# lijx10/SO-Net

Measured on AMD Instinct MI355X. Metric: point-clouds/sec forward, ModelNet40 5k-pt 8x8 SOM, higher is better.
Workload: dtype f32 (operands split into fp16 pieces, 3 fp16 MFMAs per product, f32 accumulate; parity 1e-5)

## Files before the change

### include/sonet_hip.h

```cpp
#ifndef SONET_HIP_H
#define SONET_HIP_H

#include <stddef.h>
#include <stdint.h>

#ifdef __cplusplus
extern "C" {
#endif

typedef void *sonet_stream_t;

enum {
    SONET_OK = 0,
    SONET_ERR_INVALID_ARG = 1,
    SONET_ERR_UNSUPPORTED = 2,
    SONET_ERR_LAUNCH = 3,
    SONET_ERR_NO_DEVICE = 4
};

int sonet_abi_version(void);
const char *sonet_build_arch(void);
const char *sonet_last_error(void);
int sonet_check_device(void);
int sonet_diag_mfma_f16_rate(int random_operands, int iters, double *tflops_out, double *ghz_out, sonet_stream_t stream);

int sonet_range_log_set(uint32_t *slot);

int sonet_index_max_f32(const float *data, const int32_t *index, int32_t *out_idx,
                        int B, int C, int Np, int K, sonet_stream_t stream);
int sonet_index_max_bf16(const uint16_t *data, const int32_t *index, int32_t *out_idx,
                         int B, int C, int Np, int K, sonet_stream_t stream);
int sonet_index_max_gather_f32(const float *data, const int32_t *index, const int32_t *row_max,
                               int32_t *out_idx, float *out_val,
                               int B, int C, int Np, int K, sonet_stream_t stream);
int sonet_index_max_gather_bf16(const uint16_t *data, const int32_t *index, const int32_t *row_max,
                                int32_t *out_idx, float *out_val, int B, int C, int Np, int K,
                                sonet_stream_t stream);
int sonet_index_max_gather_p16(const void *planes, const int32_t *index, const int32_t *row_max,
                               int32_t *out_idx, float *out_val, int B, int C, int Np, int K, sonet_stream_t stream);

int sonet_som_assign_f32(const float *x, const float *node, int B, int N, int M, int k,
                         int32_t *min_idx_i32, int64_t *min_idx_i64, int32_t *count, double *sum_ws,
                         sonet_stream_t stream);

int sonet_som_group_f32(const float *x, const float *sn, const int32_t *min_idx_i32,
                        const int32_t *count, const double *sum_ws, int B, int N, int M, int k,
                        float *som_node, int32_t *row_max, float *centers, float *x_decentered,
                        float *x_augmented, sonet_stream_t stream);

#define SONET_SOM_TRAIN_MAX_NODES 1024
#define SONET_SOM_TRAIN_MAX_POINTS (1 << 28)
int sonet_som_train_f32(const float *x, const float *node0, int node0_shared, const float *w, const float *lr,
                        int T, int B, int N, int M, float *node_out, sonet_stream_t stream);

int sonet_som_mask_i32(const int32_t *min_idx_i32, int32_t *mask, int B, int kN, int M,
                       sonet_stream_t stream);

int sonet_node_gather_f32(const float *feat, const int32_t *min_idx_i32, float *out,
                          int B, int C, int M, int kN, sonet_stream_t stream);

int sonet_knn_gather_f32(const float *x, const int64_t *knn_I, float *out,
                         int B, int C, int M, int K, sonet_stream_t stream);

int sonet_knn_self_f32(const float *node, int64_t *knn_I, int B, int M, int K, sonet_stream_t stream);

#define SONET_BATCH_SHAPENET 1
#define SONET_BATCH_TRAIN 2
#define SONET_BATCH_ROT_HORIZONTAL 4
#define SONET_BATCH_ROT_PERTURBATION 8
#define SONET_BATCH_TRANSLATION 16
#define SONET_BATCH_FLAG_MASK 31
#define SONET_BATCH_DRAW_SCALARS 8
#define SONET_BATCH_MAX_K 16
int sonet_assemble_batch_f32(const float *src, long long P, const int64_t *offsets, int S, const float *nodes_src,
                             const int64_t *idx, int B, int N, int M, int K, int flags, long long seed,
                             long long step, const int64_t *replay_idx, const double *replay_draws, double *draws_out,
                             float *pc, float *sn, float *node, int64_t *chosen, int64_t *knn_I, int32_t *bad,
                             sonet_stream_t stream);

int sonet_knn_group_f32(const float *coord, const float *feat, const int64_t *knn_I, int B, int C, int M, int K,
                        int center_avg, float *center, float *out, sonet_stream_t stream);
int sonet_knn_prepare_f32(const float *coord, const int64_t *knn_I, int B, int M, int K, int center_avg,
                          float *center, float *dec, int32_t *gidx, sonet_stream_t stream);
int sonet_pointmlp_h3_gather_f32(const float *x1, int C1, int L1, const int32_t *gidx, const float *x2, int C2, const void *Wp3,
                                 const float *scale, const float *shift, int relu, float *y,
                                 int B, int Cout, int L, sonet_stream_t stream);
int sonet_planes_max_f32(const float *x, float *out, long long rows, int K, int M, sonet_stream_t stream);

int sonet_lastdim_max_f32(const float *x, float *out, long long rows, int K, sonet_stream_t stream);

size_t sonet_pointmlp_pack_size(int Cin, int Cout);
int sonet_pointmlp_pack_f32(const float *W, float *Wp, int Cin, int Cout, sonet_stream_t stream);
int sonet_pointmlp_f32(const float *x1, int C1, const float *x2, int C2, const float *Wp,
                       const float *scale, const float *shift, int relu, float *y,
                       int B, int Cout, int L, sonet_stream_t stream);

int sonet_pointmlp_x3_bnb_f32(const float *gy, const float *raw, int C, const void *Wp3, const float *scale, const float *shift,
                              const float *a, const float *b, const float *c0, const float *sc, const float *sh, int relu,
                              float *g_raw_out, float *y, int B, int Cout, int L,
                              const float *praw, const float *psc, const float *psh, int prelu, void *pstats_ws, double *psums,
                              sonet_stream_t stream);

int sonet_pointmlp_x3_bnb_acc_f32(const float *gy, const float *raw, int C, const void *Wp3, const float *scale, const float *shift,
                                  const float *a, const float *b, const float *c0, const float *sc, const float *sh, int relu,
                                  float *g_raw_out, const float *yadd, float *y, int B, int Cout, int L, sonet_stream_t stream);

size_t sonet_pointmlp_x3_pack_size(int Cin, int Cout);
int sonet_pointmlp_x3_pack(const float *W, void *Wp3, int Cin, int Cout, sonet_stream_t stream);
int sonet_pointmlp_x3_f32(const float *x1, int C1, const float *x2, int C2, const void *Wp3,
                          const float *scale, const float *shift, int relu, float *y,
                          int B, int Cout, int L, sonet_stream_t stream);

int sonet_pointmlp_h3_pack(const float *W, void *Wp3, int Cin, int Cout, sonet_stream_t stream);
int sonet_pointmlp_h3_f32(const float *x1, int C1, const float *x2, int C2, const void *Wp3,
                          const float *scale, const float *shift, int relu, float *y,
                          int B, int Cout, int L, sonet_stream_t stream);

size_t sonet_p16_size(int B, int C, int L);
int sonet_p16_from_f32(const float *x, void *p16, int B, int C, int L, const float *scale, const float *shift, int relu,
                       sonet_stream_t stream);
int sonet_p16_to_f32(const void *p16, float *x, int B, int C, int L, sonet_stream_t stream);
size_t sonet_pointmlp_h3p_pack_size(int Cin, int Cout);
int sonet_pointmlp_h3p_pack(const float *W, void *Wp, int Cin, int Cout, sonet_stream_t stream);
size_t sonet_pointmlp_h3p_stats_ws_size(int B, int Cout, int L);
int sonet_pointmlp_h3p(const void *x1p, int C1, int L1, const int32_t *gidx, const void *x2p, int C2, const void *Wp,
                       const float *scale, const float *shift, int relu, float *y, void *yp, int B, int Cout, int L,
                       const float *zadd, const int32_t *zidx, int ZM, void *stats_ws, float *mean, float *var,
                       sonet_stream_t stream);

size_t sonet_knn_stage_columns(int B, int M, int K);
size_t sonet_node_stage_columns(int B, int M);
int sonet_knn_stage_prepare_f32(const float *coord, const int64_t *knn_I, int KI, int center_avg, int B, int M, int K,
                                float *center, void *center_p16, void *rec, sonet_stream_t stream);
int sonet_knn_stage_input_p16(const void *rec, const void *z_p16, const float *wl, const float *scale, const float *shift, int relu,
                              int B, int M, int K, int C, void *h1_p16, sonet_stream_t stream);
int sonet_pointmlp_h3p_gmax(const void *x1p, int C1, const void *x2p, int C2, const void *Wp, const float *scale, const float *shift,
                            int relu, int Cout, int L, int GK, int G, int ngout, int Lout, float *y, void *yp, sonet_stream_t stream);
int sonet_p16_flat_to_bcm_f32(const void *p16, float *x, int B, int C, int M, sonet_stream_t stream);

int sonet_lastdim_argmax_f32(const float *x, float *out, int32_t *idx, long long rows, int K, sonet_stream_t stream);
int sonet_lastdim_argmax_bf16(const uint16_t *x, uint16_t *out, int32_t *idx, long long rows, int K, sonet_stream_t stream);
int sonet_lastdim_max_bwd_f32(const float *g, const int32_t *idx, float *gx, long long rows, int K, sonet_stream_t stream);
int sonet_lastdim_max_bwd_bf16(const uint16_t *g, const int32_t *idx, uint16_t *gx, long long rows, int K, sonet_stream_t stream);
size_t sonet_knn_gather_bwd_ws_size(int B, int M, int K);
int sonet_knn_gather_bwd_f32(const float *g, const int64_t *knn_I, float *gx, void *ws, int B, int C, int M, int K, sonet_stream_t stream);
int sonet_knn_gather_bwd_bf16(const uint16_t *g, const int64_t *knn_I, float *gx, void *ws, int B, int C, int M, int K, sonet_stream_t stream);
size_t sonet_node_gather_bwd_ws_size(int B, int M, int L);
int sonet_node_gather_bwd_f32(const float *g, const int32_t *ids, float *gx, void *ws, int B, int C, int M, int L, sonet_stream_t stream);
int sonet_node_gather_bwd_bf16(const uint16_t *g, const int32_t *ids, float *gx, void *ws, int B, int C, int M, int L, sonet_stream_t stream);

size_t sonet_pointmlp_bf16_pack_size(int Cin, int Cout);
int sonet_pointmlp_bf16_pack(const float *W, void *Wp, int Cin, int Cout, sonet_stream_t stream);
int sonet_pointmlp_bf16(const uint16_t *x1, int C1, const uint16_t *x2, int C2, const void *Wp,
                        const float *scale, const float *shift, int relu, uint16_t *y,
                        int B, int Cout, int L, sonet_stream_t stream);
int sonet_pointmlp_bf16_gather(const uint16_t *x1, int C1, int L1, const int32_t *gidx, const uint16_t *x2, int C2, const void *Wp,
                               const float *scale, const float *shift, int relu, uint16_t *y,
                               int B, int Cout, int L, sonet_stream_t stream);
int sonet_pointmlp_bf16_acc(const uint16_t *x1, int C1, const uint16_t *x2, int C2, const void *Wp,
                            const float *scale, const float *shift, int relu, const uint16_t *yadd, uint16_t *y,
                            int B, int Cout, int L, sonet_stream_t stream);
int sonet_pointmlp_bf16_bnb(const uint16_t *gy, const uint16_t *raw, int C, const void *Wp, const float *scale, const float *shift,
                            const float *a, const float *b, const float *c0, const float *sc, const float *sh, int relu,
                            uint16_t *g_raw_out, const uint16_t *yadd, uint16_t *y, int B, int Cout, int L, sonet_stream_t stream);

size_t sonet_pointresnet_pack_size(void);
int sonet_pointresnet_pack(const float *W1, const float *W2, const float *W3, const float *W4, int Cin0,
                           void *wstream, sonet_stream_t stream);
int sonet_pointresnet_fused_f32(const float *x, int Cin0, const void *wstream, const float *affine,
                                float *y, int B, int L, sonet_stream_t stream);
int sonet_pointresnet_fused_p16_f32(const float *x, int Cin0, const void *wstream, const float *affine,
                                    float *y, void *yp, int B, int L, sonet_stream_t stream);

size_t sonet_pointresnet_bf16_pack_size(void);
int sonet_pointresnet_bf16_pack(const float *W1, const float *W2, const float *W3, const float *W4, int Cin0,
                                void *wstream, sonet_stream_t stream);
int sonet_pointresnet_bf16(const float *x, int Cin0, const void *wstream, const float *affine,
                           uint16_t *y, int B, int L, sonet_stream_t stream);

size_t sonet_pointresnet_bf16_pool_ws_size(int B, int L, int M);
int sonet_pointresnet_bf16_pool(const float *x_sorted, int Cin0, const void *wstream, const float *affine,
                                const int32_t *ids_sorted, const int32_t *pos0, const int32_t *node_off,
                                const int32_t *count, void *ws, float *out, int B, int L, int M, sonet_stream_t stream);

size_t sonet_pointresnet_pool_ws_size(int B, int L, int M);
int sonet_pointresnet_fused_pool_f32(const float *x_sorted, int Cin0, const void *wstream, const float *affine,
                                     const int32_t *ids_sorted, const int32_t *pos0, const int32_t *node_off,
                                     const int32_t *count, void *ws, float *out, int B, int L, int M, sonet_stream_t stream);
int sonet_pointresnet_fused_pool_p16_f32(const float *x_sorted, int Cin0, const void *wstream, const float *affine,
                                         const int32_t *ids_sorted, const int32_t *pos0, const int32_t *node_off,
                                         const int32_t *count, void *ws, float *out, void *out_p16, int B, int L, int M, sonet_stream_t stream);
size_t sonet_som_assign_sort_ws_size(int B, int N, int M, int k);
int sonet_som_assign_sort_f32(const float *x, const float *sn, const float *node, int B, int N, int M, int k,
                              int32_t *min_idx_i32, int64_t *min_idx_i64, int32_t *count, double *sum_ws,
                              float *som_node, int32_t *row_max, float *x_aug_sorted, int32_t *ids_sorted,
                              int32_t *pos0, int32_t *node_off, void *ws, sonet_stream_t stream);
int sonet_som_assign_sort_det_f32(const float *x, const float *sn, const float *node, int B, int N, int M, int k,
                              int32_t *min_idx_i32, int64_t *min_idx_i64, int32_t *count, double *sum_ws,
                              float *som_node, int32_t *row_max, float *x_aug_sorted, int32_t *ids_sorted,
                              int32_t *pos0, int32_t *node_off, void *ws, sonet_stream_t stream);
int sonet_som_assign_sort_knn_f32(const float *x, const float *sn, const float *node, int B, int N, int M, int k,
                                  int32_t *min_idx_i32, int64_t *min_idx_i64, int32_t *count, double *sum_ws,
                                  float *som_node, int32_t *row_max, float *x_aug_sorted, int32_t *ids_sorted,
                                  int32_t *pos0, int32_t *node_off, void *ws,
                                  const int64_t *knn_I, int KI, int K, int center_avg, float *center, void *center_p16, void *rec,
                                  sonet_stream_t stream);
int sonet_som_sort_group_f32(const float *x, const float *sn, const int32_t *min_idx_i32, const int32_t *count,
                             const double *sum_ws, int B, int N, int M, int k, float *som_node, int32_t *row_max,
                             float *x_aug_sorted, int32_t *ids_sorted, int32_t *pos0, int32_t *node_off,
                             int32_t *cursor_ws, sonet_stream_t stream);

int sonet_channel_stats_bf16(const uint16_t *y, int B, int C, int L, double *stat_ws, float *mean, float *var, sonet_stream_t stream);
int sonet_channel_affine_act_out_bf16(const uint16_t *x, const float *scale, const float *shift, int relu, uint16_t *y,
                                      int B, int C, int L, sonet_stream_t stream);
int sonet_pointwise_bwd_stats_bf16(const uint16_t *gy, const uint16_t *raw, const float *scale, const float *shift,
                                   int relu, int B, int C, int L, double *sums, sonet_stream_t stream);
int sonet_pointwise_bwd_apply_bf16(const uint16_t *gy, const uint16_t *raw, const float *scale, const float *shift, int relu,
                                   const float *a, const float *b, const float *c0, uint16_t *g_raw, int B, int C, int L,
                                   sonet_stream_t stream);

int sonet_pointwise_bwd_stats_f32(const float *gy, const float *raw, const float *scale, const float *shift,
                                  int relu, int B, int C, int L, double *sums, sonet_stream_t stream);
int sonet_pointwise_bwd_apply_f32(const float *gy, const float *raw, const float *scale, const float *shift, int relu,
                                  const float *a, const float *b, const float *c0, float *g_raw,
                                  int B, int C, int L, sonet_stream_t stream);
int sonet_node_add_affine_act_f32(float *t, const float *z, const int32_t *min_idx_i32, const float *scale,
                                  const float *shift, int relu, int B, int C, int L, int M, sonet_stream_t stream);

size_t sonet_pointmlp_stats_ws_size(int B, int Cout, int L);
int sonet_pointmlp_h3_stats_f32(const float *x1, int C1, const float *x2, int C2, const void *Wp3, const float *scale,
                                const float *shift, int relu, float *y, int B, int Cout, int L, void *stats_ws,
                                float *mean, float *var, sonet_stream_t stream);
int sonet_pointmlp_x3_stats_f32(const float *x1, int C1, const float *x2, int C2, const void *Wp3, const float *scale,
                                const float *shift, int relu, float *y, int B, int Cout, int L, void *stats_ws,
                                float *mean, float *var, sonet_stream_t stream);

int sonet_pointmlp_h3_nodeadd_f32(const float *x1, int C1, const float *x2, int C2, const void *Wp3, const float *scale,
                                  const float *shift, int relu, float *y, int B, int Cout, int L,
                                  const float *zadd, const int32_t *zidx, int ZM, sonet_stream_t stream);

size_t sonet_pointmlp_bf16_stats_ws_size(int B, int Cout, int L);
int sonet_pointmlp_bf16_stats(const uint16_t *x1, int C1, const uint16_t *x2, int C2, const void *Wp,
                              const float *scale, const float *shift, int relu, uint16_t *y,
                              int B, int Cout, int L, void *stats_ws, float *mean, float *var, sonet_stream_t stream);
int sonet_pointmlp_bf16_pool(const uint16_t *x1, int C1, const uint16_t *x2, int C2, const void *Wp,
                             const float *scale, const float *shift, int relu, const int32_t *ids, const int32_t *row_max,
                             int32_t *out_idx, float *out_val, int B, int Cout, int L, int M, sonet_stream_t stream);
int sonet_pointmlp_bf16_stats_xaff(const uint16_t *x1, int C1, const uint16_t *x2, int C2, const void *Wp,
                                   const float *scale, const float *shift, int relu, uint16_t *y,
                                   int B, int Cout, int L, void *stats_ws, float *mean, float *var,
                                   const float *xs1, const float *xh1, const float *xs2, const float *xh2, int xrelu,
                                   sonet_stream_t stream);
int sonet_pointmlp_bf16_pool_xaff(const uint16_t *x1, int C1, const uint16_t *x2, int C2, const void *Wp,
                                  const float *scale, const float *shift, int relu, const int32_t *ids, const int32_t *row_max,
                                  int32_t *out_idx, float *out_val, int B, int Cout, int L, int M,
                                  const float *xs1, const float *xh1, const float *xs2, const float *xh2, int xrelu,
                                  sonet_stream_t stream);

size_t sonet_pointmlp_h3_segpool_ws_size(int B, int Cout, int M);
int sonet_pointmlp_h3_segpool_f32(const float *x1, int C1, const float *x2, int C2, const void *Wp3, const float *scale,
                                  const float *shift, int relu, const int32_t *ids_sorted, const int32_t *pos0,
                                  const int32_t *row_max, int M, void *ws, int32_t *out_idx, float *out_val,
                                  int B, int Cout, int L, const float *xs1, const float *xh1, const float *xs2, const float *xh2,
                                  int xrelu, sonet_stream_t stream);
int sonet_pointmlp_h3_stats_xaff_f32(const float *x1, int C1, const float *x2, int C2, const void *Wp3, const float *scale,
                                     const float *shift, int relu, float *y, int B, int Cout, int L, void *stats_ws,
                                     float *mean, float *var, const float *xs1, const float *xh1, const float *xs2, const float *xh2,
                                     int xrelu, sonet_stream_t stream);

size_t sonet_wgrad_x3_ws_size(int B, int Cout, int Cin, int L);
int sonet_wgrad_x3_f32(const float *g, const float *x, float *dw, void *ws, int B, int Cout, int Cin, int L, sonet_stream_t stream);
int sonet_wgrad_x3_xaff_f32(const float *g, const float *x, float *dw, void *ws, int B, int Cout, int Cin, int L,
                            const float *xs, const float *xh, int xrelu, sonet_stream_t stream);
size_t sonet_wgrad_bf16_ws_size(int B, int Cout, int Cin, int L);
int sonet_wgrad_bf16(const uint16_t *g, const uint16_t *x, float *dw, void *ws, int B, int Cout, int Cin, int L, sonet_stream_t stream);
int sonet_wgrad_bf16_xaff(const uint16_t *g, const uint16_t *x, float *dw, void *ws, int B, int Cout, int Cin, int L,
                          const float *xs, const float *xh, int xrelu, sonet_stream_t stream);
int sonet_node_gather_lead_affine_act_f32(const float *z, const int32_t *gidx, const float *lead, const float *wl,
                                          const float *scale, const float *shift, int relu, float *out,
                                          int B, int C, int L, int M, int NL, sonet_stream_t stream);

int sonet_node_gather_lead_affine_act_bf16(const uint16_t *z, const int32_t *gidx, const float *lead, const float *wl,
                                           const float *scale, const float *shift, int relu, uint16_t *out,
                                           int B, int C, int L, int M, int NL, sonet_stream_t stream);

int sonet_linear_act_f32(const float *x, const float *W, const float *scale, const float *shift, int relu, float *y,
                         int B, int Cin, int Cout, sonet_stream_t stream);

size_t sonet_pooled_dgrad_ws_size(int B, int C, int M, int L);
int sonet_pooled_wgrad_f32(const float *g_pooled, const int32_t *pos, const float *x, int B, int C, int M, int Ci, int L,
// ... 77 lines not shown
```

### so-net_amd/csrc/common.hpp

```cpp
#pragma once
#include <hip/hip_runtime.h>
#include <stdint.h>
#include <stdio.h>
#include <stdarg.h>
#include <stdlib.h>

#include "../../include/sonet_hip.h"

namespace sonet {

constexpr int WAVE = 64;
constexpr int NUM_XCD = 8;

char *err_buf();
int fail(int code, const char *fmt, ...);

static inline hipStream_t as_stream(sonet_stream_t s) { return reinterpret_cast<hipStream_t>(s); }

static inline int launched(const char *what) {
    hipError_t e = hipGetLastError();
    if (e != hipSuccess) return fail(SONET_ERR_LAUNCH, "%s: %s", what, hipGetErrorString(e));
    return SONET_OK;
}

#define SONET_REQUIRE(cond, ...)                                      \
    do {                                                              \
        if (!(cond)) return ::sonet::fail(SONET_ERR_INVALID_ARG, __VA_ARGS__); \
    } while (0)

uint32_t *range_log();

#ifdef SONET_VARIANTS
static inline const char *knob(const char *name) { return getenv(name); }
#else
static inline const char *knob(const char *) { return nullptr; }
#endif

static inline int ceil_div(int a, int b) { return (a + b - 1) / b; }
static inline long long ceil_div64(long long a, long long b) { return (a + b - 1) / b; }

int zero_words(void *p, size_t bytes, hipStream_t st);

int launch_stats_finalize(const double *partial, int nwg, int C, double inv_n, float *mean, float *var, hipStream_t st);

struct BnRider {
    const float *gamma, *beta;
    float eps, momentum, unbias;
    float *rmean, *rvar;
    float *invstd, *sc, *sh;
};
BnRider take_bn_rider();

}

__device__ __forceinline__ float row32_sum(float v) {
    v += __builtin_bit_cast(float, __builtin_amdgcn_update_dpp(0, __builtin_bit_cast(int, v), 0xB1, 0xF, 0xF, true));
    v += __builtin_bit_cast(float, __builtin_amdgcn_update_dpp(0, __builtin_bit_cast(int, v), 0x4E, 0xF, 0xF, true));
    v += __builtin_bit_cast(float, __builtin_amdgcn_update_dpp(0, __builtin_bit_cast(int, v), 0x141, 0xF, 0xF, true));
    v += __builtin_bit_cast(float, __builtin_amdgcn_update_dpp(0, __builtin_bit_cast(int, v), 0x140, 0xF, 0xF, true));
    v += __builtin_bit_cast(float, __builtin_amdgcn_ds_swizzle(__builtin_bit_cast(int, v), 0x401F));
    return v;
}


__device__ __forceinline__ int xcd_remap(int bid, int nwg) {
    const int q = nwg / sonet::NUM_XCD, r = nwg % sonet::NUM_XCD;
    const int xcd = bid % sonet::NUM_XCD, local = bid / sonet::NUM_XCD;
    const int base = xcd < r ? xcd * (q + 1) : r * (q + 1) + (xcd - r) * q;
    return base + local;
}

struct RangeAcc { int mp; unsigned mn; };
__device__ __forceinline__ void range_track(RangeAcc &r, float x0, float x1) {
    const int a = __float_as_int(x0), b = __float_as_int(x1);
    r.mp = max(max(r.mp, a), b);
    r.mn = max(max(r.mn, (unsigned)a), (unsigned)b);
}
__device__ __forceinline__ unsigned range_amax_bits(const RangeAcc &r) {
    const unsigned neg = (r.mn & 0x80000000u) ? (r.mn & 0x7FFFFFFFu) : 0u;
    const unsigned pos = (unsigned)r.mp;
    return pos > neg ? pos : neg;
}
__device__ __forceinline__ unsigned wave_umax(unsigned v) {
#pragma unroll
    for (int o = 32; o > 0; o >>= 1) { const unsigned t = (unsigned)__shfl_xor((int)v, o, 64); v = t > v ? t : v; }
    return v;
}
__device__ __forceinline__ void range_publish(unsigned *word, unsigned wave_max_bits, int lane) {
    if (lane == 0 && wave_max_bits > __atomic_load_n(word, __ATOMIC_RELAXED)) atomicMax(word, wave_max_bits);
}

__device__ __forceinline__ void p16_split_pair(float x0, float x1, unsigned &h, unsigned &m) {
    typedef _Float16 sonet_h2_t __attribute__((ext_vector_type(2)));
    typedef float sonet_f2_t __attribute__((ext_vector_type(2)));
    const sonet_f2_t X = {32.f * __builtin_amdgcn_fmed3f(x0, -2047.f, 2047.f), 32.f * __builtin_amdgcn_fmed3f(x1, -2047.f, 2047.f)};
    const sonet_h2_t hv = __builtin_convertvector(X, sonet_h2_t);
    const sonet_f2_t R = {X[0] - (float)hv[0], X[1] - (float)hv[1]};
    h = __builtin_bit_cast(unsigned, hv);
    m = __builtin_bit_cast(unsigned, __builtin_convertvector(R, sonet_h2_t));
}
static inline int knn_stage_groups(int K) { const int g = 128 / K; return g > 16 ? 16 : g; }
```

### so-net_amd/csrc/node_stage.hip

```cpp
#include "common.hpp"

namespace {

__device__ __forceinline__ void split_pair(float x0, float x1, unsigned &h, unsigned &m) { p16_split_pair(x0, x1, h, m); }
__device__ __forceinline__ int p16_channel(int h, int e) { return 4 * h + (e & 3) + 8 * (e >> 2); }

constexpr int KS_CPW = 4;

__global__ __launch_bounds__(256) void knn_stage_prepare_kernel(const float *__restrict__ coord, const int64_t *__restrict__ I, int KI, int avg,
                                                                 int B, int M, int K, int G, long long Lp, long long Lm,
                                                                 float *__restrict__ center, uint4 *__restrict__ center_p16, int4 *__restrict__ rec,
                                                                 unsigned *__restrict__ rlog)
{
    const long long l = (long long)blockIdx.x * 256 + threadIdx.x;
    if (l >= Lp) return;
    const int col = (int)(l & 127);
    const long long BM = (long long)B * M;
    const int g = col / K, k = col - g * K;
    const long long n = (l >> 7) * G + g;
    if (!(g < G && n < BM)) {
        rec[l] = make_int4(-2, 0, 0, 0);
        return;
    }
    const int b = (int)(n / M), m = (int)(n - (long long)b * M);
    const int64_t *Ib = I + ((long long)b * M + m) * KI;
    const float *cb = coord + (long long)b * 3 * M;
    const long long id = Ib[k];
    const bool ok = (unsigned long long)id < (unsigned long long)M;
    float d[3], ctr[3];
#pragma unroll
    for (int c = 0; c < 3; ++c) {
        const float *src = cb + c * M;
        if (avg) {
            float sum = 0.f;
            for (int kk = 0; kk < K; ++kk) {
                const long long ik = Ib[kk];
                sum += ((unsigned long long)ik < (unsigned long long)M) ? src[ik] : 0.f;
            }
            ctr[c] = sum / (float)K;
        } else {
            ctr[c] = src[m];
        }
        d[c] = (ok ? src[id] : 0.f) - ctr[c];
    }
    rec[l] = make_int4(ok ? (int)((long long)b * M + id) : -1, __float_as_int(d[0]), __float_as_int(d[1]), __float_as_int(d[2]));
    if (k == 0) {
#pragma unroll
        for (int c = 0; c < 3; ++c) center[((long long)b * 3 + c) * M + m] = ctr[c];
        unsigned h0, m0, h1v, m1;
        split_pair(ctr[0], ctr[1], h0, m0);
        split_pair(ctr[2], 0.f, h1v, m1);
        center_p16[(0 * 2 + 0) * Lm + n] = make_uint4(h0, h1v, 0u, 0u);
        center_p16[(0 * 2 + 1) * Lm + n] = make_uint4(0u, 0u, 0u, 0u);
        center_p16[(1 * 2 + 0) * Lm + n] = make_uint4(m0, m1, 0u, 0u);
        center_p16[(1 * 2 + 1) * Lm + n] = make_uint4(0u, 0u, 0u, 0u);
        if (rlog != nullptr) {
            RangeAcc xr = {0, 0u};
            range_track(xr, ctr[0], ctr[1]);
            range_track(xr, ctr[2], 0.f);
            const unsigned bits = range_amax_bits(xr);
            if (bits > __atomic_load_n(rlog + 2, __ATOMIC_RELAXED)) atomicMax(rlog + 2, bits);
        }
    }
}

typedef float ks_f2 __attribute__((ext_vector_type(2)));
typedef _Float16 ks_h2 __attribute__((ext_vector_type(2)));

constexpr int KS_MAXG = 8;

__global__ __launch_bounds__(256) void knn_stage_input_kernel(const int4 *__restrict__ rec, const uint4 *__restrict__ zp, const float *__restrict__ wl,
                                                               const float *__restrict__ scale, const float *__restrict__ shift, int relu,
                                                               int C, long long Lp, long long Lm, uint4 *__restrict__ h1, unsigned *__restrict__ rlog, int abl)
{
    __shared__ unsigned wmax[4];
    __shared__ __attribute__((aligned(16))) float coef[5][KS_MAXG * KS_CPW * 16];
    const int col = threadIdx.x & 127;
    const int hh = __builtin_amdgcn_readfirstlane((int)(threadIdx.x >> 7));
    const long long lcol = (long long)blockIdx.x * 128 + col;
    const int4 r = rec[lcol];
    const int KC = (C + 15) >> 4;
    const int ngrp = (KC + KS_CPW - 1) / KS_CPW, gstride = (int)gridDim.y;
    for (int t = threadIdx.x; t < KS_MAXG * KS_CPW * 16; t += 256) {
        const int j = t >> 6, i = (t >> 4) & 3, h = (t >> 3) & 1, e = t & 7;
        const int grp = (int)blockIdx.y + j * gstride;
        const int c = (grp * KS_CPW + i) * 16 + p16_channel(h, e);
        const bool in = grp < ngrp && c < C;
        coef[0][t] = in ? 32.f * wl[c * 3 + 0] : 0.f;
        coef[1][t] = in ? 32.f * wl[c * 3 + 1] : 0.f;
        coef[2][t] = in ? 32.f * wl[c * 3 + 2] : 0.f;
        coef[3][t] = in ? scale[c] : 0.f;
        coef[4][t] = in ? 32.f * shift[c] : 0.f;
    }
    const bool valid = r.x != -2, ok = r.x >= 0;
    const ks_f2 d0 = {__int_as_float(r.y), __int_as_float(r.y)}, d1 = {__int_as_float(r.z), __int_as_float(r.z)},
                d2 = {__int_as_float(r.w), __int_as_float(r.w)};
    RangeAcc xr = {0, 0u};
    const float lo = relu ? 0.f : -65504.f;
    const uint4 *zbase = zp + (long long)hh * Lm + (ok ? r.x : 0);
    uint4 *hbase = h1 + (long long)hh * Lp + lcol;

    auto load = [&](uint4 (&zh)[KS_CPW], uint4 (&zm)[KS_CPW], int grp) {
        const uint4 *zq = zbase + (long long)(grp * KS_CPW) * 4 * Lm;
#pragma unroll
        for (int i = 0; i < KS_CPW; ++i) {
            zh[i] = make_uint4(0u, 0u, 0u, 0u);
            zm[i] = zh[i];
#ifdef SONET_VARIANTS
            if (abl & 2) { zh[i] = make_uint4(r.y, r.z, r.w, r.x); zm[i] = zh[i]; } else
#endif
            if (ok && grp * KS_CPW + i < KC) {
                zh[i] = zq[0];
                zm[i] = zq[2 * Lm];
            }
            zq += 4 * Lm;
        }
    };
    auto process = [&](const uint4 (&zhq)[KS_CPW], const uint4 (&zmq)[KS_CPW], int grp, int j) {
        uint4 *hq = hbase + (long long)(grp * KS_CPW) * 4 * Lp;
#pragma unroll
        for (int i = 0; i < KS_CPW; ++i) {
            if (grp * KS_CPW + i >= KC) break;
            const unsigned zh[4] = {zhq[i].x, zhq[i].y, zhq[i].z, zhq[i].w}, zm[4] = {zmq[i].x, zmq[i].y, zmq[i].z, zmq[i].w};
            unsigned hv[4], mv[4];
#pragma unroll
            for (int q = 0; q < 4; ++q) {
                const int slot = (j * KS_CPW + i) * 16 + hh * 8 + 2 * q;
                const ks_f2 w0 = *reinterpret_cast<const ks_f2 *>(&coef[0][slot]), w1 = *reinterpret_cast<const ks_f2 *>(&coef[1][slot]),
                            w2 = *reinterpret_cast<const ks_f2 *>(&coef[2][slot]), sc = *reinterpret_cast<const ks_f2 *>(&coef[3][slot]),
                            sh = *reinterpret_cast<const ks_f2 *>(&coef[4][slot]);
                const ks_h2 zh2 = __builtin_bit_cast(ks_h2, zh[q]), zm2 = __builtin_bit_cast(ks_h2, zm[q]);
                ks_f2 a = __builtin_convertvector(zh2, ks_f2) + __builtin_convertvector(zm2, ks_f2);
                a = __builtin_elementwise_fma(w0, d0, a);
                a = __builtin_elementwise_fma(w1, d1, a);
                a = __builtin_elementwise_fma(w2, d2, a);
                a = __builtin_elementwise_fma(a, sc, sh);
                if (!valid) a = ks_f2{0.f, 0.f};
                range_track(xr, a[0], a[1]);
                const ks_f2 X = {__builtin_amdgcn_fmed3f(a[0], lo, 65504.f), __builtin_amdgcn_fmed3f(a[1], lo, 65504.f)};
                const ks_h2 hp = __builtin_convertvector(X, ks_h2);
                const ks_f2 R = X - __builtin_convertvector(hp, ks_f2);
                hv[q] = __builtin_bit_cast(unsigned, hp);
                mv[q] = __builtin_bit_cast(unsigned, __builtin_convertvector(R, ks_h2));
            }
#ifdef SONET_VARIANTS
            if ((abl & 1) && hv[0] != 0x12345u) { hq += 4 * Lp; continue; }
#endif
            hq[0] = make_uint4(hv[0], hv[1], hv[2], hv[3]);
            hq[2 * Lp] = make_uint4(mv[0], mv[1], mv[2], mv[3]);
            hq += 4 * Lp;
        }
    };

    uint4 zhA[KS_CPW], zmA[KS_CPW], zhB[KS_CPW], zmB[KS_CPW];
    int grp = (int)blockIdx.y, j = 0;
    load(zhA, zmA, grp);
    __syncthreads();
    for (; grp < ngrp; grp += 2 * gstride, j += 2) {
        const bool more = grp + gstride < ngrp;
        if (more) load(zhB, zmB, grp + gstride);
        process(zhA, zmA, grp, j);
        if (more) {
            if (grp + 2 * gstride < ngrp) load(zhA, zmA, grp + 2 * gstride);
            process(zhB, zmB, grp + gstride, j + 1);
        }
    }
    if (rlog != nullptr) {
        unsigned bits;
        if (relu) {
            const unsigned pos = xr.mp > 0 ? (unsigned)xr.mp : 0u, nan_neg = xr.mn > 0xFF800000u ? (xr.mn & 0x7FFFFFFFu) : 0u;
            bits = pos > nan_neg ? pos : nan_neg;
        } else {
            bits = range_amax_bits(xr);
        }
        unsigned wm = wave_umax(bits);
        wm = wm > (5u << 23) ? wm - (5u << 23) : 0u;
        if ((threadIdx.x & 63) == 0) wmax[threadIdx.x >> 6] = wm;
        __syncthreads();
        if (threadIdx.x == 0) {
            const unsigned a = wmax[0] > wmax[1] ? wmax[0] : wmax[1], c2 = wmax[2] > wmax[3] ? wmax[2] : wmax[3];
            const unsigned mx = a > c2 ? a : c2;
            if (mx > __atomic_load_n(rlog + 2, __ATOMIC_RELAXED)) atomicMax(rlog + 2, mx);
        }
    }
}

__global__ __launch_bounds__(256) void p16_flat_to_bcm_kernel(const uint4 *__restrict__ p, float *__restrict__ x, int C, int M, long long BM, long long Lm, int KC)
{
    const long long l = (long long)blockIdx.x * 256 + threadIdx.x;
    const int kc = blockIdx.y >> 1, hh = blockIdx.y & 1;
    if (l >= BM) return;
    const uint4 hv = p[((long long)(kc * 2 + 0) * 2 + hh) * Lm + l], mv = p[((long long)(kc * 2 + 1) * 2 + hh) * Lm + l];
    typedef _Float16 f16x8 __attribute__((ext_vector_type(8)));
    const f16x8 h8 = __builtin_bit_cast(f16x8, hv), m8 = __builtin_bit_cast(f16x8, mv);
    const long long b = l / M;
    const int m = (int)(l - b * M);
#pragma unroll
    for (int e = 0; e < 8; ++e) {
        const int c = kc * 16 + p16_channel(hh, e);
        if (c < C) x[(b * C + c) * M + m] = ((float)h8[e] + (float)m8[e]) * 0.03125f;
    }
}

}

extern "C" size_t sonet_knn_stage_columns(int B, int M, int K)
{
    if (B <= 0 || M <= 0 || K <= 0 || K > 128) return 0;
    return (size_t)(sonet::ceil_div64((long long)B * M, knn_stage_groups(K)) * 128);
}

extern "C" size_t sonet_node_stage_columns(int B, int M)
{
    if (B <= 0 || M <= 0) return 0;
    return (size_t)(sonet::ceil_div64((long long)B * M, 128) * 128);
}

extern "C" int sonet_knn_stage_prepare_f32(const float *coord, const int64_t *knn_I, int KI, int center_avg, int B, int M, int K,
                                           float *center, void *center_p16, void *rec, sonet_stream_t stream)
{
    const char *what = "sonet_knn_stage_prepare_f32";
    SONET_REQUIRE(coord && knn_I && center && center_p16 && rec, "%s: NULL pointer", what);
    SONET_REQUIRE(B > 0 && M > 0 && K >= 1 && K <= 128 && KI >= K, "%s: bad size B=%d M=%d K=%d (of %d)", what, B, M, K, KI);
    const long long Lp = (long long)sonet_knn_stage_columns(B, M, K), Lm = (long long)sonet_node_stage_columns(B, M);
    if (Lp / 256 + 1 > 0x7FFFFFFFll) return sonet::fail(SONET_ERR_UNSUPPORTED, "%s: too many columns", what);
    hipLaunchKernelGGL(knn_stage_prepare_kernel, dim3((unsigned)sonet::ceil_div64(Lp, 256)), dim3(256), 0, sonet::as_stream(stream),
                       coord, knn_I, KI, center_avg, B, M, K, knn_stage_groups(K), Lp, Lm, center, reinterpret_cast<uint4 *>(center_p16),
                       reinterpret_cast<int4 *>(rec), sonet::range_log());
    return sonet::launched(what);
}

extern "C" int sonet_knn_stage_input_p16(const void *rec, const void *z_p16, const float *wl, const float *scale, const float *shift, int relu,
                                         int B, int M, int K, int C, void *h1_p16, sonet_stream_t stream)
{
    const char *what = "sonet_knn_stage_input_p16";
    SONET_REQUIRE(rec && z_p16 && wl && scale && shift && h1_p16, "%s: NULL pointer", what);
    SONET_REQUIRE(B > 0 && M > 0 && C > 0 && K >= 1 && K <= 128, "%s: bad size B=%d M=%d C=%d K=%d", what, B, M, C, K);
    const long long Lp = (long long)sonet_knn_stage_columns(B, M, K), Lm = (long long)sonet_node_stage_columns(B, M);
    const long long nblk = Lp / 128;
    const int KC = sonet::ceil_div(C, 16);
    if (nblk > 0x7FFFFFFFll || (double)KC * 64.0 * (double)Lp >= 2.0e9) return sonet::fail(SONET_ERR_UNSUPPORTED, "%s: too many columns", what);
    const int ngrp = sonet::ceil_div(KC, KS_CPW);
    int gy = sonet::ceil_div(ngrp, KS_MAXG);
    while (gy < ngrp && nblk * gy < 512) ++gy;
#ifdef SONET_VARIANTS
    if (const char *e = sonet::knob("SONET_KSI_GY")) { const int v = atoi(e); if (v >= sonet::ceil_div(ngrp, KS_MAXG) && v <= ngrp) gy = v; }
#endif
    hipLaunchKernelGGL(knn_stage_input_kernel, dim3((unsigned)nblk, (unsigned)gy), dim3(256), 0, sonet::as_stream(stream),
                       reinterpret_cast<const int4 *>(rec), reinterpret_cast<const uint4 *>(z_p16), wl, scale, shift, relu, C, Lp, Lm,
                       reinterpret_cast<uint4 *>(h1_p16), sonet::range_log(), sonet::knob("SONET_KSI_ABL") ? atoi(sonet::knob("SONET_KSI_ABL")) : 0);
    return sonet::launched(what);
}

extern "C" int sonet_p16_flat_to_bcm_f32(const void *p16, float *x, int B, int C, int M, sonet_stream_t stream)
{
    const char *what = "sonet_p16_flat_to_bcm_f32";
    SONET_REQUIRE(p16 && x, "%s: NULL pointer", what);
    SONET_REQUIRE(B > 0 && C > 0 && M > 0, "%s: non-positive size", what);
    const int KC = sonet::ceil_div(C, 16);
    const long long BM = (long long)B * M;
    if (KC * 2 > 65535) return sonet::fail(SONET_ERR_UNSUPPORTED, "%s: C too large for one launch", what);
    hipLaunchKernelGGL(p16_flat_to_bcm_kernel, dim3((unsigned)sonet::ceil_div64(BM, 256), (unsigned)(KC * 2)), dim3(256), 0, sonet::as_stream(stream),
                       reinterpret_cast<const uint4 *>(p16), x, C, M, BM, (long long)sonet_node_stage_columns(B, M), KC);
    return sonet::launched(what);
}
```

### so-net_amd/csrc/pointmlp_h3p.hip

```cpp
#include "common.hpp"

namespace {

typedef float f32x16 __attribute__((ext_vector_type(16)));
typedef _Float16 f16x8 __attribute__((ext_vector_type(8)));
typedef _Float16 f16x2_t __attribute__((ext_vector_type(2)));
typedef float f32x2_t __attribute__((ext_vector_type(2)));
typedef unsigned u32x4 __attribute__((ext_vector_type(4)));
typedef int i32x4_t __attribute__((ext_vector_type(4)));

constexpr int P_THREADS = 256;
constexpr int P_KPAD = 8;
constexpr unsigned OOB = 0x7FFFFF00u;

__device__ __forceinline__ unsigned pk_f16(float lo, float hi) {
    const f32x2_t v = {lo, hi};
    return __builtin_bit_cast(unsigned, __builtin_convertvector(v, f16x2_t));
}
__device__ __forceinline__ void split2(float X0, float X1, unsigned &h, unsigned &m) {
    h = pk_f16(X0, X1);
    const f16x2_t hv = __builtin_bit_cast(f16x2_t, h);
    m = pk_f16(X0 - (float)hv[0], X1 - (float)hv[1]);
}
template <bool RELU>
__device__ __forceinline__ void split_act(float x0, float x1, unsigned &h, unsigned &m) {
    constexpr float lo = RELU ? 0.f : -2047.f;
    split2(32.f * __builtin_amdgcn_fmed3f(x0, lo, 2047.f), 32.f * __builtin_amdgcn_fmed3f(x1, lo, 2047.f), h, m);
}

__device__ __forceinline__ int p16_channel(int h, int e) { return 4 * h + (e & 3) + 8 * (e >> 2); }

__global__ __launch_bounds__(256) void h3p_pack_kernel(const float *__restrict__ W, uint4 *__restrict__ Wp, int Cin, int Cout, int KCP,
                                                        long long total, unsigned *__restrict__ trailer)
{
    const long long t = (long long)blockIdx.x * 256 + threadIdx.x;
    if (t >= total) return;
    RangeAcc wr = {0, 0u};
    const int lane = (int)(t & 63);
    const long long r = t >> 6;
    const int kc = (int)(r % KCP), ct = (int)(r / KCP);
    const int o = ct * 32 + (lane & 31), hh = lane >> 5;
    unsigned h[4], m[4];
#pragma unroll
    for (int p = 0; p < 4; ++p) {
        const int c0 = kc * 16 + p16_channel(hh, 2 * p), c1 = c0 + 1;
        float w0 = (o < Cout && c0 < Cin) ? W[(long long)o * Cin + c0] : 0.f;
        float w1 = (o < Cout && c1 < Cin) ? W[(long long)o * Cin + c1] : 0.f;
        range_track(wr, w0, w1);
        w0 = 32.f * __builtin_fminf(__builtin_fmaxf(w0, -2047.f), 2047.f);
        w1 = 32.f * __builtin_fminf(__builtin_fmaxf(w1, -2047.f), 2047.f);
        split2(w0, w1, h[p], m[p]);
    }
    uint4 *dst = Wp + (r * 2) * 64 + lane;
    dst[0] = make_uint4(h[0], h[1], h[2], h[3]);
    dst[64] = make_uint4(m[0], m[1], m[2], m[3]);
    range_publish(trailer, wave_umax(range_amax_bits(wr)), lane);
}

template <bool AFFINE>
__global__ __launch_bounds__(256) void p16_from_f32_kernel(const float *__restrict__ x, uint4 *__restrict__ p, int C, int L, int KC,
                                                            const float *__restrict__ scale, const float *__restrict__ shift, int relu,
                                                            unsigned *__restrict__ rlog)
{
    __shared__ unsigned wmax[4];
    const int kc = blockIdx.y >> 1, hh = blockIdx.y & 1, b = blockIdx.z;
    RangeAcc xr = {0, 0u};
    const float *xb0 = x + (size_t)b * C * L;
    uint4 *pb = p + (size_t)b * KC * 4 * L;
    float sc[8], sf[8];
    if constexpr (AFFINE) {
#pragma unroll
        for (int e = 0; e < 8; ++e) {
            const int c = kc * 16 + p16_channel(hh, e);
            sc[e] = c < C ? scale[c] : 0.f;
            sf[e] = c < C ? shift[c] : 0.f;
        }
    }
#pragma unroll
    for (int it = 0; it < 4; ++it) {
        const int l = blockIdx.x * 1024 + it * 256 + threadIdx.x;
        if (l >= L) break;
        const float *xb = xb0 + l;
        float v[8];
#pragma unroll
        for (int e = 0; e < 8; ++e) {
            const int c = kc * 16 + p16_channel(hh, e);
            float t = c < C ? xb[(size_t)c * L] : 0.f;
            if constexpr (AFFINE) {
                t = __fmaf_rn(t, sc[e], sf[e]);
                if (relu) t = t < 0.f ? 0.f : t;
            }
            v[e] = t;
        }
        unsigned h[4], m[4];
#pragma unroll
        for (int q = 0; q < 4; ++q) {
            range_track(xr, v[2 * q], v[2 * q + 1]);
            split_act<false>(v[2 * q], v[2 * q + 1], h[q], m[q]);
        }
        pb[((size_t)(kc * 2 + 0) * 2 + hh) * L + l] = make_uint4(h[0], h[1], h[2], h[3]);
        pb[((size_t)(kc * 2 + 1) * 2 + hh) * L + l] = make_uint4(m[0], m[1], m[2], m[3]);
    }
    if (rlog != nullptr) {
        const unsigned wm = wave_umax(range_amax_bits(xr));
        if ((threadIdx.x & 63) == 0) wmax[threadIdx.x >> 6] = wm;
        __syncthreads();
        if (threadIdx.x == 0) {
            const unsigned a = wmax[0] > wmax[1] ? wmax[0] : wmax[1], c2 = wmax[2] > wmax[3] ? wmax[2] : wmax[3];
            const unsigned mx = a > c2 ? a : c2;
            if (mx > __atomic_load_n(rlog + 2, __ATOMIC_RELAXED)) atomicMax(rlog + 2, mx);
        }
    }
}

__global__ __launch_bounds__(256) void p16_to_f32_kernel(const uint4 *__restrict__ p, float *__restrict__ x, int C, int L, int KC)
{
    const int l = blockIdx.x * 256 + threadIdx.x;
    const int kc = blockIdx.y >> 1, hh = blockIdx.y & 1, b = blockIdx.z;
    if (l >= L) return;
    const uint4 *pb = p + (size_t)b * KC * 4 * L;
    const uint4 hv = pb[((size_t)(kc * 2 + 0) * 2 + hh) * L + l], mv = pb[((size_t)(kc * 2 + 1) * 2 + hh) * L + l];
    const f16x8 h8 = __builtin_bit_cast(f16x8, hv), m8 = __builtin_bit_cast(f16x8, mv);
    float *xb = x + (size_t)b * C * L + l;
#pragma unroll
    for (int e = 0; e < 8; ++e) {
        const int c = kc * 16 + p16_channel(hh, e);
        if (c < C) xb[(size_t)c * L] = ((float)h8[e] + (float)m8[e]) * 0.03125f;
    }
}

struct H3pArgs {
    const void *x1, *x2;
    const void *Wp;
    const float *scale, *shift;
    float *y;
    void *yp;
    const int32_t *gidx;
    const float *zadd;
    const int32_t *zidx;
    unsigned *rlog;
    double *stats_partial;
    int abl;
    unsigned long long *prof;
    long long ngroups;
    int KC1, KC2, L1, L, Cout, CT, KC, KCr, KCP, ct_per_y, nslab, ncol, gpc, relu, ZM;
    int GK, G, ngout, Lout;
};

__device__ __forceinline__ i32x4_t make_rsrc(const void *base, unsigned bytes) {
    const unsigned long long a = reinterpret_cast<unsigned long long>(base);
    i32x4_t r;
    r[0] = __builtin_amdgcn_readfirstlane((int)(unsigned)a);
    r[1] = __builtin_amdgcn_readfirstlane((int)(unsigned)((a >> 32) & 0xFFFFu));
    r[2] = __builtin_amdgcn_readfirstlane((int)bytes);
    r[3] = 0x00020000;
    return r;
}
__device__ __forceinline__ u32x4 bload16(i32x4_t rsrc, unsigned voff, unsigned soff) {
    u32x4 r;
    asm volatile("buffer_load_dwordx4 %0, %1, %2, %3 offen" : "=v"(r) : "v"(voff), "s"(rsrc), "s"(soff) : "memory");
    return r;
}
__device__ __forceinline__ void bstore16(__amdgpu_buffer_rsrc_t rsrc, unsigned voff, unsigned soff, u32x4 v) {
    __builtin_amdgcn_raw_buffer_store_b128(v, rsrc, voff, soff, 0);
}
__device__ __forceinline__ void bstore4(__amdgpu_buffer_rsrc_t rsrc, unsigned voff, unsigned soff, float v) {
    __builtin_amdgcn_raw_buffer_store_b32(__builtin_bit_cast(unsigned, v), rsrc, voff, soff, 0);
}
template <int N>
__device__ __forceinline__ void wait_barrier(u32x4 &a, u32x4 &b) {
    asm volatile("s_waitcnt vmcnt(%2)\n\ts_barrier" : "+v"(a), "+v"(b) : "n"(N) : "memory");
}
template <int N>
__device__ __forceinline__ void wait_barrier(u32x4 &a, u32x4 &b, u32x4 &c, u32x4 &d) {
    asm volatile("s_waitcnt vmcnt(%4)\n\ts_barrier" : "+v"(a), "+v"(b), "+v"(c), "+v"(d) : "n"(N) : "memory");
}

template <int NC>
__device__ __forceinline__ void sched_pair() {
    __builtin_amdgcn_sched_group_barrier(0x100, 1, 0);
    __builtin_amdgcn_sched_group_barrier(0x008, NC == 2 ? 3 : 1, 0);
    __builtin_amdgcn_sched_group_barrier(0x100, 1, 0);
    __builtin_amdgcn_sched_group_barrier(0x008, NC == 2 ? 3 : 2, 0);
    __builtin_amdgcn_sched_group_barrier(0x100, 1, 0);
    __builtin_amdgcn_sched_group_barrier(0x008, NC == 2 ? 3 : 1, 0);
    __builtin_amdgcn_sched_group_barrier(0x100, 1, 0);
    __builtin_amdgcn_sched_group_barrier(0x008, NC == 2 ? 3 : 2, 0);
}

constexpr int GM_STRIDE = 136;
__device__ __forceinline__ float nan_max(float m, float v) { return (v > m || v != v) ? v : m; }
__device__ __forceinline__ void lds_barrier() { asm volatile("s_waitcnt lgkmcnt(0)\n\ts_barrier" ::: "memory"); }

template <int MT, int NC, int OCC, int EPI, int OUT>
__global__ __launch_bounds__(P_THREADS, OCC) void pointmlp_h3p_kernel(const H3pArgs a)
{
    static_assert(OUT >= 1 && OUT <= 3 && (EPI != 2 || (OUT & 1)), "output mode");
    static_assert(EPI < 4 || (NC == 1 && ((EPI == 4 && OUT == 2) || (EPI == 5 && OUT == 1))), "group-max epilogues: 32-column waves, P16 (4) or f32 (5) out");
    static_assert(MT % 2 == 0 && (NC == 1 || NC == 2), "tile shape");
    constexpr int PB = (OCC >= 2 && NC == 2 && (EPI == 1 || EPI == 3)) ? 2 : 3, NB = 4, D = 3, NSLOT = D + 2;
    static_assert(D >= PB && PB >= 2, "the wait count below assumes the W request of a chunk is older than its X request");
    constexpr int NSL = MT * 2;
    constexpr int ND = NSL / 4;
    constexpr int NBL = NC * 2;
    constexpr int NP = MT / 2;
    constexpr int KWAIT = (PB - 1) * (NBL + ND);
    static_assert(KWAIT < 64, "vmcnt is a 6-bit counter");
    struct Lds {
        u32x4 wsm[NSLOT][NSL][64];
        float aff[EPI == 1 ? 1024 : 2048];
        float2 red[EPI == 2 ? 4 : 1][EPI == 2 ? MT * 32 : 1];
        float zl[EPI == 1 ? MT * 32 : 1][EPI == 1 ? 64 : 1];
        float gm[EPI >= 4 ? 32 : 1][EPI >= 4 ? GM_STRIDE : 1];
    };
    __shared__ __attribute__((aligned(16))) Lds lds;

    const int wg_xcd = blockIdx.x & 7, wg_local = blockIdx.x >> 3;
    const int wg_col = (wg_local / a.nslab) * 8 + wg_xcd, wg_slab = wg_local - (wg_local / a.nslab) * a.nslab;
    if (wg_col >= a.ncol) return;

    const int lane = threadIdx.x & 63;
    const int wave = __builtin_amdgcn_readfirstlane(threadIdx.x >> 6);
    const int j = lane & 31, h = lane >> 5;
    long long q = (long long)wg_col * 4 + wave;
    const bool wave_valid = q < a.ngroups;
    q = wave_valid ? q : 0;
    const int b = __builtin_amdgcn_readfirstlane((int)(q / a.gpc));
    const int l0 = __builtin_amdgcn_readfirstlane((int)(q - (long long)b * a.gpc) * (32 * NC));
    const int L = a.L, L1 = a.L1;

    bool pv[NC];
    unsigned vo1[NC], vo2[NC], voy[NC], voyp[NC];
    int lcl[NC];
#pragma unroll
    for (int c = 0; c < NC; ++c) {
        const int l = l0 + 32 * c + j;
        pv[c] = wave_valid && l < L;
        lcl[c] = l < L ? l : l0;
        vo2[c] = (unsigned)(h * L + lcl[c]) * 16u;
        vo1[c] = (unsigned)(h * L1 + lcl[c]) * 16u;
        if (a.gidx) {
            const int src = a.gidx[(size_t)b * L + lcl[c]];
            vo1[c] = (unsigned)src < (unsigned)L1 ? (unsigned)(h * L1 + src) * 16u : OOB;
        }
        voy[c] = pv[c] ? (unsigned)(4 * h * L + l) * 4u : OOB;
        voyp[c] = pv[c] ? (unsigned)(h * L + l) * 16u : OOB;
#ifdef SONET_VARIANTS
        if (a.abl & 1) { voy[c] = OOB; voyp[c] = OOB; pv[c] = false; }
#endif
    }
    const i32x4_t r1 = make_rsrc(static_cast<const char *>(a.x1) + (size_t)b * a.KC1 * 64 * L1, (unsigned)a.KC1 * 64u * (unsigned)L1);
    const i32x4_t r2 = make_rsrc(a.x2 ? static_cast<const char *>(a.x2) + (size_t)b * a.KC2 * 64 * L : static_cast<const char *>(a.x1),
                                 a.x2 ? (unsigned)a.KC2 * 64u * (unsigned)L : 0u);
    const __amdgpu_buffer_rsrc_t ry = __builtin_amdgcn_make_buffer_rsrc(
        a.y ? reinterpret_cast<char *>(a.y) + (size_t)b * a.Cout * L * 4 : nullptr, 0, a.y ? (int)((unsigned)a.Cout * (unsigned)L * 4u) : 0, 0x00020000);
    const __amdgpu_buffer_rsrc_t ryp = __builtin_amdgcn_make_buffer_rsrc(
        a.yp ? static_cast<char *>(a.yp) + (size_t)b * (a.Cout / 16) * 64 * L : nullptr, 0, a.yp ? (int)((unsigned)(a.Cout / 16) * 64u * (unsigned)L) : 0, 0x00020000);

    const int ct_begin = wg_slab * a.ct_per_y;
    const int ct_end = min(a.CT, ct_begin + a.ct_per_y);
    const int npass = (ct_end - ct_begin) / MT;
    const int KCr = a.KCr, KC1 = a.KC1;
#ifdef SONET_VARIANTS
    unsigned long long pt0 = __builtin_readcyclecounter(), pt_loop = 0, pt_epi = 0, pt_pro = 0;
#endif
    const unsigned wsm_lds = (unsigned)reinterpret_cast<size_t>(&lds.wsm[0][0][0]);
    const unsigned vow = (unsigned)lane * 16u;
    const char *wp = static_cast<const char *>(a.Wp);

    auto load_b = [&](u32x4 (&bb)[NBL], int kc) {
#ifdef SONET_VARIANTS
        if (a.abl & 2) kc = 0;
#endif
        const bool second = kc >= KC1;
        const int kk = second ? kc - KC1 : kc;
        const unsigned rowb = (unsigned)(second ? L : L1) * 32u;
        const i32x4_t rs = second ? r2 : r1;
#pragma unroll
        for (int c = 0; c < NC; ++c) {
            const unsigned vo = second ? vo2[c] : vo1[c];
            bb[2 * c + 0] = bload16(rs, vo, (unsigned)(kk * 2 + 0) * rowb);
            bb[2 * c + 1] = bload16(rs, vo, (unsigned)(kk * 2 + 1) * rowb);
        }
    };
    auto dma = [&](int pass, int kc, int slot) {
#ifdef SONET_VARIANTS
        if (a.abl & 4) { kc = 0; pass = 0; }
#endif
        const int ps = pass < npass ? pass : npass - 1;
        const char *g0 = wp + ((size_t)(ct_begin + ps * MT) * a.KCP + kc) * 2048u;
        const unsigned d0 = wsm_lds + (unsigned)slot * (unsigned)(NSL * 1024);
#pragma unroll
        for (int t = 0; t < ND; ++t) {
            const int sl = wave + 4 * t;
            const char *g = g0 + (size_t)(sl >> 1) * ((size_t)a.KCP * 2048u) + (size_t)(sl & 1) * 1024u;
            const unsigned d = d0 + (unsigned)sl * 1024u;
            unsigned keep;
            asm volatile("s_mov_b32 %0, m0\n\ts_mov_b32 m0, %3\n\ts_nop 4\n\tglobal_load_lds_dwordx4 %1, %2\n\ts_mov_b32 m0, %0"
                         : "=&s"(keep) : "v"(vow), "s"(g), "s"(d) : "memory");
        }
    };
    auto read_a = [&](u32x4 (&A)[4], int slot, int p) {
#pragma unroll
        for (int u = 0; u < 4; ++u) A[u] = lds.wsm[slot][4 * p + u][lane];
    };

    f32x16 acc[MT][NC];

    auto mfma_pair = [&](const u32x4 (&A)[4], const u32x4 (&bb)[NBL], int p) {
        f16x8 Bh[NC], Bm[NC];
#pragma unroll
        for (int c = 0; c < NC; ++c) {
            Bh[c] = __builtin_bit_cast(f16x8, bb[2 * c + 0]);
            Bm[c] = __builtin_bit_cast(f16x8, bb[2 * c + 1]);
        }
#pragma unroll
        for (int term = 0; term < 3; ++term)
#pragma unroll
            for (int tt = 0; tt < 2; ++tt)
#pragma unroll
                for (int c = 0; c < NC; ++c)
                {
                    const f16x8 wf = __builtin_bit_cast(f16x8, A[2 * tt + (term == 0 ? 1 : 0)]), xf = term == 1 ? Bm[c] : Bh[c];
                    acc[2 * p + tt][c] = __builtin_amdgcn_mfma_f32_32x32x16_f16(wf, xf, acc[2 * p + tt][c], 0, 0, 0);
                }
    };

    RangeAcc yr = {0, 0u};
    const float relu_thr = a.relu ? 0.f : -__builtin_inff();
    const float split_lo = a.relu ? 0.f : -2047.f;
    int zm[NC];
    bool zok[NC];
    unsigned zvo[NC], zla[NC];
    const i32x4_t rz = make_rsrc(a.zadd ? a.zadd + (size_t)b * a.Cout * a.ZM : nullptr, a.zadd ? (unsigned)a.Cout * (unsigned)a.ZM * 4u : 0u);
    if constexpr (EPI == 1 || EPI == 3) {
#pragma unroll
        for (int c = 0; c < NC; ++c) {
            zm[c] = a.zidx[(size_t)b * L + lcl[c]];
            zok[c] = (unsigned)zm[c] < (unsigned)a.ZM;
            zm[c] = zok[c] ? zm[c] : 0;
            zvo[c] = zok[c] ? (unsigned)(zm[c] + 4 * h * a.ZM) * 4u : OOB;
            zla[c] = (unsigned)reinterpret_cast<size_t>(&lds.zl[4 * h][zm[c]]);
            asm volatile("" : "+v"(zla[c]));
        }
    }
    auto epilogue = [&](int ct0) {
        if constexpr (EPI >= 4) {
#pragma unroll
            for (int mt = 0; mt < MT; ++mt) {
                if ((ct0 + mt) * 32 >= a.Cout) continue;
                float asc16[16], ash16[16];
                {
                    const float4 *t4 = reinterpret_cast<const float4 *>(lds.aff + (ct0 - ct_begin + mt) * 64 + h * 32);
#pragma unroll
                    for (int u = 0; u < 4; ++u) {
                        const float4 s4 = t4[u], h4 = t4[4 + u];
                        asc16[4 * u] = s4.x; asc16[4 * u + 1] = s4.y; asc16[4 * u + 2] = s4.z; asc16[4 * u + 3] = s4.w;
                        ash16[4 * u] = h4.x; ash16[4 * u + 1] = h4.y; ash16[4 * u + 2] = h4.z; ash16[4 * u + 3] = h4.w;
                    }
                }
                __builtin_amdgcn_sched_barrier(0);
#pragma unroll
                for (int r = 0; r < 16; ++r) {
                    const float v = __fmaf_rn(acc[mt][0][r], asc16[r], ash16[r]);
                    lds.gm[(r & 3) + 8 * (r >> 2) + 4 * h][32 * wave + j] = v < relu_thr ? 0.f : v;
                }
                lds_barrier();
                const int t = (int)threadIdx.x;
                if constexpr (EPI == 4) {
                    const int p = t & 3, u = t >> 2;
                    const int g = u % a.G, qh = u / a.G;
                    if (qh < 4) {
                        const int qq = qh >> 1, h2 = qh & 1;
                        const float *r0 = &lds.gm[16 * qq + 4 * h2 + 2 * (p & 1) + 8 * (p >> 1)][g * a.GK];
                        float m0 = r0[0], m1 = r0[GM_STRIDE];
                        for (int k = 1; k < a.GK; ++k) {
                            m0 = nan_max(m0, r0[k]);
                            m1 = nan_max(m1, r0[GM_STRIDE + k]);
                        }
                        const long long n_out = (long long)wg_col * a.G + g;
                        if (n_out < a.ngout) {
                            range_track(yr, m0, m1);
                            unsigned hv, mv;
                            split2(__builtin_amdgcn_fmed3f(m0, split_lo * 32.f, 65504.f), __builtin_amdgcn_fmed3f(m1, split_lo * 32.f, 65504.f), hv, mv);
                            unsigned *dst = reinterpret_cast<unsigned *>(static_cast<char *>(a.yp)
                                + ((((size_t)((ct0 + mt) * 2 + qq) * 2) * 2 + h2) * (size_t)a.Lout + (size_t)n_out) * 16) + p;
                            dst[0] = hv;
                            dst[(size_t)a.Lout * 8] = mv;
                        }
                    }
                } else {
                    const int seg = t & 3, row = (t >> 2) & 31, g = t >> 7;
                    const int cols = a.GK >> 2;
                    const float *r0 = &lds.gm[row][(g < a.G ? g : 0) * a.GK + seg * cols];
                    float m = r0[0];
                    for (int k = 1; k < cols; ++k) m = nan_max(m, r0[k]);
                    m = nan_max(m, __builtin_bit_cast(float, __builtin_amdgcn_update_dpp(0, __builtin_bit_cast(int, m), 0xB1, 0xF, 0xF, true)));
                    m = nan_max(m, __builtin_bit_cast(float, __builtin_amdgcn_update_dpp(0, __builtin_bit_cast(int, m), 0x4E, 0xF, 0xF, true)));
                    const long long n_out = (long long)wg_col * a.G + g;
                    if (seg == 0 && g < a.G && n_out < a.ngout) a.y[(size_t)n_out * a.Cout + (size_t)(ct0 + mt) * 32 + row] = m;
                }
                lds_barrier();
            }
            return;
        }
#pragma unroll
        for (int mt = 0; mt < MT; ++mt) {
            if ((ct0 + mt) * 32 >= a.Cout) continue;
            float asc16[16], ash16[16];
            {
                const float4 *t4 = reinterpret_cast<const float4 *>(lds.aff + (ct0 - ct_begin + mt) * 64 + h * 32);
#pragma unroll
                for (int u = 0; u < 4; ++u) {
                    const float4 s4 = t4[u], h4 = t4[4 + u];
                    asc16[4 * u] = s4.x; asc16[4 * u + 1] = s4.y; asc16[4 * u + 2] = s4.z; asc16[4 * u + 3] = s4.w;
                    ash16[4 * u] = h4.x; ash16[4 * u + 1] = h4.y; ash16[4 * u + 2] = h4.z; ash16[4 * u + 3] = h4.w;
                }
            }
            __builtin_amdgcn_sched_barrier(0);
            float st1[EPI == 2 ? 16 : 1], st2[EPI == 2 ? 16 : 1];
#pragma unroll
            for (int c = 0; c < NC; ++c) {
#pragma unroll
                for (int qq = 0; qq < 2; ++qq) {
                    unsigned hh[4], mm[4];
#pragma unroll
                    for (int hf = 0; hf < 2; ++hf) {
                        const int r0 = 8 * qq + 4 * hf;
                        const int row0 = mt * 32 + 16 * qq + 8 * hf;
                        float av[4], v[4], zg[4];
#pragma unroll
                        for (int e = 0; e < 4; ++e) {
                            if constexpr (OCC == 1) asm volatile("v_accvgpr_read_b32 %0, %1" : "=v"(av[e]) : "a"(acc[mt][c][r0 + e]));
                            else av[e] = acc[mt][c][r0 + e];
                        }
                        if constexpr (EPI == 3) {
#pragma unroll
                            for (int e = 0; e < 4; ++e) {
                                const unsigned so = (unsigned)((ct0 + mt) * 32 + 16 * qq + 8 * hf + e) * (unsigned)a.ZM * 4u;
                                asm volatile("buffer_load_dword %0, %1, %2, %3 offen" : "=v"(zg[e]) : "v"(zvo[c]), "s"(rz), "s"(so) : "memory");
                            }
                            asm volatile("s_waitcnt vmcnt(0)" : "+v"(zg[0]), "+v"(zg[1]), "+v"(zg[2]), "+v"(zg[3]) :: "memory");
                        }
                        if constexpr (EPI == 1) {
#pragma unroll
                            for (int e = 0; e < 4; ++e)
                                asm volatile("v_add_u32 %0, %2, %1\n\tds_read_b32 %0, %0" : "=&v"(zg[e]) : "v"(zla[c]), "s"((row0 + e) * 256) : "memory");
                            asm volatile("s_waitcnt lgkmcnt(0)" : "+v"(zg[0]), "+v"(zg[1]), "+v"(zg[2]), "+v"(zg[3]) :: "memory");
                        }
#pragma unroll
                        for (int e = 0; e < 4; ++e) {
                            const float sc = asc16[r0 + e], sf = ash16[r0 + e];
                            if constexpr (EPI == 1 || EPI == 3) {
                                const float zv = EPI == 1 ? (zok[c] ? zg[e] : 0.f) : zg[e];
                                v[e] = __fmaf_rn(av[e], sc, __fmaf_rn(zv, sc * 1024.f, sf));
                            } else {
                                v[e] = __fmaf_rn(av[e], sc, sf);
                            }
                        }
                        if constexpr ((OUT & 1) != 0) {
#pragma unroll
                            for (int e = 0; e < 4; ++e) {
                                const int orow = 16 * qq + 8 * hf + e;
                                const float o = v[e] < relu_thr ? 0.f : v[e];
                                bstore4(ry, voy[c], (unsigned)((ct0 + mt) * 32 + orow) * (unsigned)L * 4u, o);
                                if constexpr (EPI == 2) {
                                    const float vv = pv[c] ? o : 0.f;
                                    st1[r0 + e] = c == 0 ? vv : st1[r0 + e] + vv;
                                    st2[r0 + e] = c == 0 ? vv * vv : st2[r0 + e] + vv * vv;
                                }
                            }
                        }
                        if constexpr ((OUT & 2) != 0) {
#pragma unroll
                            for (int p = 0; p < 2; ++p) {
                                const float x0 = v[2 * p], x1 = v[2 * p + 1];
                                range_track(yr, x0, x1);
                                if constexpr (OUT == 2)
                                    split2(__builtin_amdgcn_fmed3f(x0, split_lo * 32.f, 65504.f), __builtin_amdgcn_fmed3f(x1, split_lo * 32.f, 65504.f),
                                           hh[2 * hf + p], mm[2 * hf + p]);
                                else
                                    split2(32.f * __builtin_amdgcn_fmed3f(x0, split_lo, 2047.f), 32.f * __builtin_amdgcn_fmed3f(x1, split_lo, 2047.f),
                                           hh[2 * hf + p], mm[2 * hf + p]);
                            }
                        }
                        if constexpr (EPI == 1 || EPI == 3 || OUT == 3) __builtin_amdgcn_sched_barrier(0);
                    }
                    if constexpr ((OUT & 2) == 0) __builtin_amdgcn_sched_barrier(0);
                    if constexpr ((OUT & 2) != 0) {
                        const unsigned so = (unsigned)(((ct0 + mt) * 2 + qq) * 2) * (unsigned)L * 32u;
                        const u32x4 hv = {hh[0], hh[1], hh[2], hh[3]}, mv = {mm[0], mm[1], mm[2], mm[3]};
                        bstore16(ryp, voyp[c], so, hv);
                        bstore16(ryp, voyp[c], so + (unsigned)L * 32u, mv);
                        __builtin_amdgcn_sched_barrier(0);
                    }
                }
            }
            if constexpr (EPI == 2) {
#pragma unroll
                for (int r = 0; r < 16; ++r) {
                    const float s1 = row32_sum(st1[r]), s2 = row32_sum(st2[r]);
                    if (j == 0) lds.red[wave][mt * 32 + (r & 3) + 8 * (r >> 2) + 4 * h] = make_float2(s1, s2);
                }
                __builtin_amdgcn_sched_barrier(0);
            }
        }
        if constexpr (EPI == 2) {
            __syncthreads();
            for (int t = threadIdx.x; t < MT * 32 && ct0 * 32 + t < a.Cout; t += P_THREADS) {
                const double s = ((double)lds.red[0][t].x + (double)lds.red[1][t].x) + ((double)lds.red[2][t].x + (double)lds.red[3][t].x);
                const double qq = ((double)lds.red[0][t].y + (double)lds.red[1][t].y) + ((double)lds.red[2][t].y + (double)lds.red[3][t].y);
                double *dst = a.stats_partial + ((size_t)wg_col * a.Cout + (size_t)ct0 * 32 + t) * 2;
                dst[0] = s;
                dst[1] = qq;
            }
            __syncthreads();
        }
        if constexpr (EPI == 1) __syncthreads();
    };
    auto z_dma = [&](int ct0) {
        if constexpr (EPI == 1) {
            {
                const char *g0 = reinterpret_cast<const char *>(a.zadd + ((size_t)b * a.Cout + (size_t)ct0 * 32) * 64);
                const unsigned d0 = (unsigned)reinterpret_cast<size_t>(&lds.zl[0][0]);
#pragma unroll
                for (int t = 0; t < MT * 2; ++t) {
                    const int piece = wave + 4 * t;
                    const char *g = g0 + (size_t)piece * 1024u;
                    const unsigned d = d0 + (unsigned)piece * 1024u;
                    unsigned keep;
                    asm volatile("s_mov_b32 %0, m0\n\ts_mov_b32 m0, %3\n\ts_nop 4\n\tglobal_load_lds_dwordx4 %1, %2\n\ts_mov_b32 m0, %0"
                                 : "=&s"(keep) : "v"(vow), "s"(g), "s"(d) : "memory");
                }
            }
        }
    };

    u32x4 bq[NB][NBL];
    u32x4 Aq[2][4];
#pragma unroll
    for (int i = 0; i <= D - PB; ++i) dma(0, i, i);
#pragma unroll
    for (int t = -PB; t <= -2; ++t) {
        load_b(bq[(t + PB) & 3], t + PB);
        dma(0, t + 1 + D, t + 1 + D);
    }
    load_b(bq[(PB - 1) & 3], PB - 1);
    if constexpr (NBL == 2) wait_barrier<KWAIT>(bq[0][0], bq[0][1]);
    else wait_barrier<KWAIT>(bq[0][0], bq[0][1], bq[0][2], bq[0][3]);
    dma(0, D, D);
    read_a(Aq[0], 0, 0);
    for (int o = ct_begin * 32 + (int)threadIdx.x; o < ct_end * 32; o += P_THREADS)
    {
        const int rel = o - ct_begin * 32, rr = rel & 31;
        constexpr float pre = OUT == 2 ? 32.f : 1.f;
        const float scv = o < a.Cout ? a.scale[o] * (pre / 1024.f) : 0.f, shv = o < a.Cout ? a.shift[o] * pre : 0.f;
        float *t = lds.aff + (rel >> 5) * 64 + ((rr >> 2) & 1) * 32 + ((rr & 3) | ((rr >> 3) << 2));
        t[0] = scv;
        t[16] = shv;
    }
    __syncthreads();
#ifdef SONET_VARIANTS
    pt_pro = __builtin_readcyclecounter() - pt0;
#endif

    int kcb = PB;
    int kcd = (1 + D) % KCr, passd = (1 + D) / KCr;
    int slot = 0;
    if (kcb >= KCr) kcb -= KCr;

#define H3P_BODY(I)                                                                                                   \
    {                                                                                                                 \
        load_b(bq[((I) + PB) & 3], kcb);                                                                              \
        const int slot1 = slot + 1 < NSLOT ? slot + 1 : 0;                                                            \
        int slotd = slot + 1 + D;                                                                                     \
        slotd = slotd >= NSLOT ? slotd - NSLOT : slotd;                                                               \
        _Pragma("unroll") for (int p = 0; p < NP; ++p) {                                                              \
            constexpr int base_par = ((I) * NP) & 1;                                                                  \
            const int cur = (base_par + p) & 1;                                                                       \
            if (p == NP - 1) {                                                                                        \
                if constexpr (NBL == 2) wait_barrier<KWAIT>(bq[((I) + 1) & 3][0], bq[((I) + 1) & 3][1]);              \
                else wait_barrier<KWAIT>(bq[((I) + 1) & 3][0], bq[((I) + 1) & 3][1], bq[((I) + 1) & 3][2], bq[((I) + 1) & 3][3]); \
                dma(passd, kcd, slotd);                                                                               \
                read_a(Aq[cur ^ 1], slot1, 0);                                                                        \
            } else {                                                                                                  \
                read_a(Aq[cur ^ 1], slot, p + 1);                                                                     \
            }                                                                                                         \
            mfma_pair(Aq[cur], bq[(I)], p);                                                                           \
             \
            sched_pair<NC>();                                                                                         \
        }                                                                                                             \
        slot = slot1;                                                                                                 \
        kcb = kcb + 1 < KCr ? kcb + 1 : 0;                                                                            \
        if (kcd + 1 < KCr) kcd += 1; else { kcd = 0; passd += 1; }                                                    \
    }

    for (int pass = 0; pass < npass; ++pass) {
#pragma unroll
        for (int mt = 0; mt < MT; ++mt)
#pragma unroll
            for (int c = 0; c < NC; ++c)
#pragma unroll
                for (int r = 0; r < 16; ++r) acc[mt][c][r] = 0.f;
        z_dma(ct_begin + pass * MT);
#ifdef SONET_VARIANTS
        const unsigned long long pl0 = __builtin_readcyclecounter();
#endif
        for (int k4 = 0; k4 < KCr; k4 += 4) {
            H3P_BODY(0)
            H3P_BODY(1)
            H3P_BODY(2)
            H3P_BODY(3)
        }
#ifdef SONET_VARIANTS
        const unsigned long long pl1 = __builtin_readcyclecounter();
        pt_loop += pl1 - pl0;
#endif
#ifdef SONET_VARIANTS
        if (!(a.abl & 8))
#endif
        epilogue(ct_begin + pass * MT);
#ifdef SONET_VARIANTS
        pt_epi += __builtin_readcyclecounter() - pl1;
#endif
    }
#undef H3P_BODY
    asm volatile("s_waitcnt vmcnt(0)" ::: "memory");
#ifdef SONET_VARIANTS
    if (a.prof != nullptr && threadIdx.x == 0) {
        atomicAdd(a.prof + 0, 1ull);
        atomicAdd(a.prof + 1, pt_pro);
        atomicAdd(a.prof + 2, pt_loop);
        atomicAdd(a.prof + 3, pt_epi);
        atomicAdd(a.prof + 4, (unsigned long long)__builtin_readcyclecounter() - pt0);
    }
#endif

    if (a.rlog != nullptr) {
        if (a.yp) {
            const unsigned pos = yr.mp > 0 ? (unsigned)yr.mp : 0u, nan_neg = yr.mn > 0xFF800000u ? (yr.mn & 0x7FFFFFFFu) : 0u;
            unsigned bits = wave_umax(a.relu ? (pos > nan_neg ? pos : nan_neg) : range_amax_bits(yr));
            if constexpr (OUT == 2) bits = bits > (5u << 23) ? bits - (5u << 23) : 0u;
            range_publish(a.rlog + 2, bits, lane);
        }
        if (ct_begin == 0 && wg_col == 0 && threadIdx.x == 0)
            atomicMax(a.rlog + 1, reinterpret_cast<const unsigned *>(wp + (size_t)a.CT * a.KCP * 2048u)[0]);
    }
}

}


extern "C" size_t sonet_p16_size(int B, int C, int L)
{
    if (B <= 0 || C <= 0 || L <= 0) return 0;
    return (size_t)B * (size_t)sonet::ceil_div(C, 16) * 64 * (size_t)L;
}

extern "C" int sonet_p16_from_f32(const float *x, void *p16, int B, int C, int L, const float *scale, const float *shift, int relu,
                                  sonet_stream_t stream)
{
    const char *what = "sonet_p16_from_f32";
    SONET_REQUIRE(x && p16, "%s: NULL pointer", what);
    SONET_REQUIRE(B > 0 && C > 0 && L > 0, "%s: non-positive size", what);
    SONET_REQUIRE((scale == nullptr) == (shift == nullptr), "%s: scale and shift come together", what);
    const int KC = sonet::ceil_div(C, 16);
    if (B > 65535 || KC * 2 > 65535) return sonet::fail(SONET_ERR_UNSUPPORTED, "%s: B or C too large for one launch", what);
    dim3 grid((unsigned)sonet::ceil_div(L, 1024), (unsigned)(KC * 2), (unsigned)B);
    unsigned *rlog = sonet::range_log();
    if (scale) hipLaunchKernelGGL(p16_from_f32_kernel<true>, grid, dim3(256), 0, sonet::as_stream(stream), x, reinterpret_cast<uint4 *>(p16), C, L, KC, scale, shift, relu, rlog);
    else       hipLaunchKernelGGL(p16_from_f32_kernel<false>, grid, dim3(256), 0, sonet::as_stream(stream), x, reinterpret_cast<uint4 *>(p16), C, L, KC, scale, shift, relu, rlog);
    return sonet::launched(what);
}

extern "C" int sonet_p16_to_f32(const void *p16, float *x, int B, int C, int L, sonet_stream_t stream)
{
    const char *what = "sonet_p16_to_f32";
    SONET_REQUIRE(x && p16, "%s: NULL pointer", what);
    SONET_REQUIRE(B > 0 && C > 0 && L > 0, "%s: non-positive size", what);
    const int KC = sonet::ceil_div(C, 16);
    if (B > 65535 || KC * 2 > 65535) return sonet::fail(SONET_ERR_UNSUPPORTED, "%s: B or C too large for one launch", what);
    dim3 grid((unsigned)sonet::ceil_div(L, 256), (unsigned)(KC * 2), (unsigned)B);
    hipLaunchKernelGGL(p16_to_f32_kernel, grid, dim3(256), 0, sonet::as_stream(stream), reinterpret_cast<const uint4 *>(p16), x, C, L, KC);
    return sonet::launched(what);
}

extern "C" size_t sonet_pointmlp_h3p_pack_size(int Cin, int Cout)
{
    if (Cin <= 0 || Cout <= 0) return 0;
    const size_t kcp = (size_t)sonet::ceil_div(Cin, 16 * P_KPAD) * P_KPAD;
    return (size_t)(sonet::ceil_div(Cout, 64) * 2) * kcp * 2048 + 64;
}

extern "C" int sonet_pointmlp_h3p_pack(const float *W, void *Wp, int Cin, int Cout, sonet_stream_t stream)
{
    const char *what = "sonet_pointmlp_h3p_pack";
    SONET_REQUIRE(W && Wp, "%s: NULL pointer", what);
    SONET_REQUIRE(Cin > 0 && Cout > 0, "%s: non-positive size", what);
    const int KCP = sonet::ceil_div(Cin, 16 * P_KPAD) * P_KPAD;
    const long long total = (long long)(sonet::ceil_div(Cout, 64) * 2) * KCP * 64;
    unsigned *trailer = reinterpret_cast<unsigned *>(reinterpret_cast<uint4 *>(Wp) + total * 2);
    if (sonet::zero_words(trailer, 64, sonet::as_stream(stream)) != 0) return sonet::fail(SONET_ERR_LAUNCH, "%s: clearing the trailer failed", what);
    hipLaunchKernelGGL(h3p_pack_kernel, dim3((unsigned)sonet::ceil_div64(total, 256)), dim3(256), 0, sonet::as_stream(stream),
                       W, reinterpret_cast<uint4 *>(Wp), Cin, Cout, KCP, total, trailer);
    return sonet::launched(what);
}

extern "C" size_t sonet_pointmlp_h3p_stats_ws_size(int B, int Cout, int L)
{
    if (B <= 0 || Cout <= 0 || L <= 0) return 0;
    return (size_t)sonet::ceil_div64((long long)B * sonet::ceil_div(L, 32), 4) * Cout * 2 * sizeof(double);
}

namespace {
struct Shape { int MT, NC, OCC; };

template <int MT, int NC, int OCC>
int launch_shape(int epi, int out, unsigned nwg, hipStream_t st, const H3pArgs &a)
{
#define H3P_GO(E, O) hipLaunchKernelGGL((pointmlp_h3p_kernel<MT, NC, OCC, E, O>), dim3(nwg), dim3(P_THREADS), 0, st, a)
    if (epi == 2 && out == 1) H3P_GO(2, 1);
    else if (epi == 1 && out == 1) { if constexpr (MT <= 8) H3P_GO(1, 1); else return 1; }
    else if (epi == 1 && out == 2) { if constexpr (MT <= 8) H3P_GO(1, 2); else return 1; }
    else if (epi == 3 && out == 1) H3P_GO(3, 1);
    else if (epi == 3 && out == 2) H3P_GO(3, 2);
    else if (epi == 0 && out == 1) H3P_GO(0, 1);
    else if (epi == 0 && out == 2) H3P_GO(0, 2);
    else if (epi == 0 && out == 3) H3P_GO(0, 3);
    else if (epi == 4 && out == 2) { if constexpr (NC == 1) H3P_GO(4, 2); else return 1; }
    else if (epi == 5 && out == 1) { if constexpr (NC == 1) H3P_GO(5, 1); else return 1; }
    else return 1;
#undef H3P_GO
    return 0;
}
}

static int h3p_launch(const char *what, const void *x1p, int C1, int L1, const int32_t *gidx, const void *x2p, int C2, const void *Wp,
                      const float *scale, const float *shift, int relu, float *y, void *yp, int B, int Cout, int L,
                      const float *zadd, const int32_t *zidx, int ZM, void *stats_ws, float *mean, float *var,
                      int GK, int G, int ngout, int Lout, sonet_stream_t stream)
{
    if (!gidx) L1 = L;
    SONET_REQUIRE(x1p && Wp && scale && shift && (y || yp), "%s: NULL pointer", what);
    SONET_REQUIRE(B > 0 && C1 > 0 && C2 >= 0 && Cout > 0 && L > 0 && L1 > 0, "%s: non-positive size", what);
    SONET_REQUIRE((C2 == 0) == (x2p == nullptr), "%s: x2 and C2 disagree", what);
    SONET_REQUIRE(C2 == 0 || C1 % 16 == 0, "%s: with a second input C1=%d must be a multiple of 16", what, C1);
    SONET_REQUIRE((zadd == nullptr) == (zidx == nullptr) && (!zadd || ZM > 0), "%s: zadd, zidx and ZM come together", what);
    SONET_REQUIRE(!stats_ws || (y && !yp && mean && var && !zadd), "%s: the statistics epilogue needs y (only), mean, var and no addend", what);
    if (Cout % 32 != 0) return sonet::fail(SONET_ERR_UNSUPPORTED, "%s: Cout=%d must be a multiple of 32", what, Cout);
    const int KC1 = sonet::ceil_div(C1, 16), KC2 = sonet::ceil_div(C2, 16), KC = KC1 + KC2;
    const int KCP = sonet::ceil_div(C1 + C2, 16 * P_KPAD) * P_KPAD;
    const int KCr = sonet::ceil_div(KC, 4) * 4;
    const int CT = sonet::ceil_div(Cout, 64) * 2;
    if ((double)KC1 * 64.0 * L1 >= 2.0e9 || (double)KC2 * 64.0 * L >= 2.0e9 || (double)Cout * L * 4.0 >= 2.0e9 || (double)CT * KCP * 2048.0 >= 2.0e9)
        return sonet::fail(SONET_ERR_UNSUPPORTED, "%s: a per-cloud panel exceeds 2 GiB", what);
    const long long cols = (long long)B * L;
    Shape sh = (CT % 4 == 0) ? ((cols >= 131072 && GK == 0) ? Shape{4, 2, 2} : Shape{4, 1, 2}) : Shape{2, 1, 2};
#ifdef SONET_VARIANTS
    if (const char *e = sonet::knob("SONET_H3P_SHAPE")) {
        int m = 0, n = 0, o = 0;
        if (sscanf(e, "%d,%d,%d", &m, &n, &o) == 3 && CT % m == 0) sh = Shape{m, n, o};
    }
#endif
    const int gpc = sonet::ceil_div(L, 32 * sh.NC);
    const long long ngroups = (long long)B * gpc, ncol = sonet::ceil_div64(ngroups, 4);
    const int groups = CT / sh.MT;
    int nslab = 1;
    for (int d = 1; d <= groups; ++d)
        if (groups % d == 0 && (d <= 4 || cols < 131072 || CT / nslab > (zadd ? 16 : 32))) nslab = d;
#ifdef SONET_VARIANTS
    if (const char *e = sonet::knob("SONET_H3P_NSLAB")) {
        const int want = atoi(e);
        if (want >= 1 && groups % want == 0 && CT / want <= 32) nslab = want;
    }
#endif
    const long long nwg = sonet::ceil_div64(ncol, 8) * 8 * nslab;
    if (nwg > 0x7FFFFFFFll || ncol > 0x7FFFFFFFll) return sonet::fail(SONET_ERR_UNSUPPORTED, "%s: too many points", what);
    if (stats_ws && sonet::ceil_div64((long long)B * sonet::ceil_div(L, 32), 4) < ncol)
        return sonet::fail(SONET_ERR_UNSUPPORTED, "%s: statistics workspace too small", what);
    H3pArgs a;
    a.x1 = x1p; a.x2 = x2p; a.Wp = Wp; a.scale = scale; a.shift = shift; a.y = y; a.yp = yp; a.gidx = gidx; a.zadd = zadd; a.zidx = zidx;
    a.rlog = sonet::range_log(); a.stats_partial = reinterpret_cast<double *>(stats_ws); a.ngroups = ngroups;
    a.prof = nullptr; a.abl = 0;
#ifdef SONET_VARIANTS
    if (const char *e = sonet::knob("SONET_H3P_ABL")) a.abl = atoi(e);
    if (const char *e = sonet::knob("SONET_H3P_PROF")) a.prof = reinterpret_cast<unsigned long long *>(strtoull(e, nullptr, 0));
#endif
    a.KC1 = KC1; a.KC2 = KC2; a.L1 = L1; a.L = L; a.Cout = Cout; a.CT = CT; a.KC = KC; a.KCr = KCr; a.KCP = KCP; a.ct_per_y = CT / nslab;
    a.nslab = nslab; a.ncol = (int)ncol; a.gpc = gpc; a.relu = relu; a.ZM = ZM;
    a.GK = GK; a.G = G; a.ngout = ngout; a.Lout = Lout;
    hipStream_t st = sonet::as_stream(stream);
    const int epi = GK ? (yp ? 4 : 5)
                       : stats_ws ? 2 : zadd ? ((ZM == 64 && gpc % 4 == 0 && CT / nslab <= 16 && Cout % 64 == 0) ? 1 : 3) : 0;
    const unsigned g = (unsigned)nwg;
    const int out = (y ? 1 : 0) | (yp ? 2 : 0);
    int miss = 1;
    if (sh.MT == 4 && sh.NC == 2) miss = launch_shape<4, 2, 2>(epi, out, g, st, a);
    else if (sh.MT == 4 && sh.NC == 1) miss = launch_shape<4, 1, 2>(epi, out, g, st, a);
    else if (sh.MT == 2 && sh.NC == 1) miss = launch_shape<2, 1, 2>(epi, out, g, st, a);
#ifdef SONET_VARIANTS
    else if (sh.MT == 8 && sh.NC == 2) miss = launch_shape<8, 2, 1>(epi, out, g, st, a);
    else if (sh.MT == 6 && sh.NC == 2) miss = launch_shape<6, 2, 1>(epi, out, g, st, a);
    else if (sh.MT == 12 && sh.NC == 1) miss = launch_shape<12, 1, 1>(epi, out, g, st, a);
#endif
    if (miss) return sonet::fail(SONET_ERR_UNSUPPORTED, "%s: no kernel for tile shape %d x %d with epilogue %d and outputs %d", what, sh.MT, sh.NC, epi, out);
    if (stats_ws) sonet::launch_stats_finalize(reinterpret_cast<const double *>(stats_ws), (int)ncol, Cout, 1.0 / ((double)B * L), mean, var, st);
    return sonet::launched(what);
}

extern "C" int sonet_pointmlp_h3p(const void *x1p, int C1, int L1, const int32_t *gidx, const void *x2p, int C2, const void *Wp,
                                  const float *scale, const float *shift, int relu, float *y, void *yp, int B, int Cout, int L,
                                  const float *zadd, const int32_t *zidx, int ZM, void *stats_ws, float *mean, float *var,
                                  sonet_stream_t stream)
{
    return h3p_launch("sonet_pointmlp_h3p", x1p, C1, L1, gidx, x2p, C2, Wp, scale, shift, relu, y, yp, B, Cout, L, zadd, zidx, ZM, stats_ws, mean, var,
                      0, 0, 0, 0, stream);
}

extern "C" int sonet_pointmlp_h3p_gmax(const void *x1p, int C1, const void *x2p, int C2, const void *Wp, const float *scale, const float *shift,
                                       int relu, int Cout, int L, int GK, int G, int ngout, int Lout, float *y, void *yp, sonet_stream_t stream)
{
    const char *what = "sonet_pointmlp_h3p_gmax";
    SONET_REQUIRE((y == nullptr) != (yp == nullptr), "%s: exactly one of y (f32 [ngout][Cout]) and yp (P16 planes)", what);
    SONET_REQUIRE(L > 0 && L % 128 == 0, "%s: L=%d must be a positive multiple of 128", what, L);
    SONET_REQUIRE(GK >= 1 && G >= 1 && G * GK <= 128 && ngout >= 1 && (long long)ngout <= (long long)(L / 128) * G, "%s: bad grouping GK=%d G=%d ngout=%d", what, GK, G, ngout);
    SONET_REQUIRE(!yp || Lout >= ngout, "%s: Lout=%d (the planes' column count) below ngout=%d", what, Lout, ngout);
    if (yp) { if (G > 16) return sonet::fail(SONET_ERR_UNSUPPORTED, "%s: at most 16 groups per 128 columns for P16 output (G=%d)", what, G); }
    else if (G > 2 || GK % 4 != 0) return sonet::fail(SONET_ERR_UNSUPPORTED, "%s: f32 output takes G <= 2 groups of GK %% 4 == 0 columns (G=%d GK=%d)", what, G, GK);
    return h3p_launch(what, x1p, C1, L, nullptr, x2p, C2, Wp, scale, shift, relu, y, yp, 1, Cout, L, nullptr, nullptr, 0, nullptr, nullptr, nullptr,
                      GK, G, ngout, Lout, stream);
}
```

### so-net_amd/models/networks.py

```python
import math

import weakref

import torch
import torch.nn as nn

from sonet_hip import ops as _ops
from util import som
from .layers import EquivariantLayer, KNNModule, MyLinear, PointNet, PointResNet, _PlainAttrs


def _head_inference(fn):
    import functools

    @functools.wraps(fn)
    def wrapper(self, *args, **kwargs):
        ts = [a for a in args if isinstance(a, torch.Tensor) and a.is_floating_point()]
        dev = ts[0].device if ts else torch.device("cpu")
        if torch.is_grad_enabled() and not self.training and getattr(self, "inference", True):
            if ts and not any(t.requires_grad for t in ts) and any(getattr(t, "_sonet_inference", False) for t in ts):
                with torch.no_grad():
                    return _ops.mark_inference(_ops.run_guarded(lambda: fn(self, *args, **kwargs), dev, True))
        return _ops.run_guarded(lambda: fn(self, *args, **kwargs), dev, not (torch.is_grad_enabled() or self.training))
    return wrapper
# ... 49 lines not shown
            self.knnlayer = KNNModule(3 + 384, (512, 512), activation=act, normalization=norm, **kw)
            self.final_pointnet = PointNet(3 + 512, (768, self.feature_num), activation=act, normalization=norm, **kw)
        else:
            self.final_pointnet = PointResNet(3 + 384, (512, 512, 768, self.feature_num),
                                              activation=act, normalization=norm, **kw)
        rows = int(math.sqrt(opt.node_num))
        self.som_builder = som.BatchSOM(rows, rows, 3, opt.gpu_id, opt.batch_size)
        self.zero_pad = torch.nn.ZeroPad2d(padding=1)
        self._lazy = None
        self._first_pn_out = None

    @property
    def mask(self):
        st = self._lazy
        if st is None:
            raise AttributeError("Encoder.mask: call forward first")
        if st.get("mask") is None:
            st["mask"] = _ops.som_mask(st["a"].min_idx_i32, st["a"].M)
        return st["mask"]

    @property
    def min_idx(self):
        st = self._lazy
        if st.get("min_idx") is None:
            st["min_idx"] = st["a"].min_idx_i32.long()
        return st["min_idx"]

    def _per_point(self, name):
        st = self._lazy
        if st is None:
            raise AttributeError("Encoder.%s: call forward first" % name)
        if st.get(name) is None:
            g = _ops.som_group(st["x"], None, st["a"], want_centers=True, want_decentered=True)
            st["centers"], st["x_decentered"] = g["centers"], g["x_decentered"]
        return _ops.mark_inference(st[name]) if getattr(self, "_infer_tag", False) else st[name]

    @property
    def first_pn_out(self):
        if self._first_pn_out is None and self._lazy is not None and self._lazy.get("first_p16") is not None:
            self._first_pn_out = self._lazy["first_p16"].float()
        if self._first_pn_out is None and self._lazy is not None and self._lazy.get("not_materialised"):
            raise RuntimeError("Encoder.first_pn_out was not materialised by this training forward (only its per-node maximum is consumed: the "
                               "pool ran in the last layer's epilogue); set encoder.want_first_pn_out = True before the forward to keep it")
        if self._first_pn_out is None and self._lazy is not None:
            st = self._lazy
            g = _ops.som_group(st["x"], st["sn"], st["a"], want_augmented=st["sn"] is not None, want_decentered=st["sn"] is None)
            with torch.no_grad():
                self._first_pn_out = self.first_pointnet(g["x_augmented"] if st["sn"] is not None else g["x_decentered"], None)
        if getattr(self, "_infer_tag", False):
            _ops.mark_inference(self._first_pn_out)
        return self._first_pn_out

    @first_pn_out.setter
    def first_pn_out(self, v):
        self._first_pn_out = v

    def _stage_map(self, name):
        v = self.__dict__.get("_" + name)
        st = self.__dict__.get("_stage")
        if v is None and st is not None:
            with torch.no_grad():
                if name == "knn_feature_1":
                    v = _ops.p16_flat_to_bcm(st["knn_p16"], st["B"], st["M"])
                else:
                    lyr = self.final_pointnet.layers[1]
                    sc, sh = lyr._eval_affine()
                    y = _ops.pointmlp_h3p(st["h3_p16"], lyr._packed_p16(), sc, sh, lyr.activation == 'relu', lyr.conv.out_channels, out="f32")
                    v = y[0, :, :st["B"] * st["M"]].reshape(-1, st["B"], st["M"]).permute(1, 0, 2).contiguous()
            if getattr(self, "_infer_tag", False):
                _ops.mark_inference(v)
            self.__dict__["_" + name] = v
        return v

    @property
    def knn_feature_1(self):
        return self._stage_map("knn_feature_1")

    @knn_feature_1.setter
    def knn_feature_1(self, v):
        self.__dict__["_knn_feature_1"] = v

    @property
    def final_pn_out(self):
        return self._stage_map("final_pn_out")

    @final_pn_out.setter
    def final_pn_out(self, v):
        self.__dict__["_final_pn_out"] = v

    @property
    def centers(self):
        return self._per_point("centers")

    @property
    def x_decentered(self):
        return self._per_point("x_decentered")

    def forward(self, x, sn, node=None, node_knn_I=None, is_train=False, epoch=None):
        if node is None or node_knn_I is None:
            node, node_knn_I = self._raw_cloud_nodes(x, node, node_knn_I)
        infer = (not is_train) and (not self.training) and getattr(self, "inference", True) and not x.requires_grad
        if infer and torch.is_grad_enabled():
            with torch.no_grad():
                out = self._forward_guarded(x, sn, node, node_knn_I, is_train, epoch)
        else:
            out = self._forward_guarded(x, sn, node, node_knn_I, is_train, epoch)
        self._infer_tag = (not torch.is_grad_enabled()) or infer
        if self._infer_tag:
            for t in (out, self.first_pn_out_masked_max, self.__dict__.get("_final_pn_out"), self.som_node, self.__dict__.get("_knn_feature_1")):
                _ops.mark_inference(t)
        return out

    def _raw_cloud_nodes(self, x, node, node_knn_I):
        with torch.no_grad():
            if node is None:
                self.som_builder.optimize(x.detach())
                node = self.som_builder.node
            if node_knn_I is None:
                node_knn_I = _ops.knn_self(node.detach().float().contiguous(), int(self.opt.som_k))
        return node, node_knn_I

    def _wants_dense(self):
        v = self.__dict__.get('want_first_pn_out')
        return bool(v) if v is not None else len(_DENSE_HEADS) > 0

    def _node_stage_ok(self, B, M, node_knn_I):
        opt = self.opt
        if not (_ops.NODE_STAGE_P16 and _ops.GATHER_NODE_STAGE and _ops.P16_CHAINS and _ops.POINTMLP_PRECISION == "h3" and opt.som_k >= 2) \
                or torch.is_grad_enabled():
            return False
        if getattr(self, 'want_first_pn_out', False):
            return False
        if M not in (64, 128) or node_knn_I is None or node_knn_I.dim() != 3 or node_knn_I.dtype != torch.int64 \
                or node_knn_I.shape[2] < opt.som_k or opt.som_k > 128 or opt.som_k_type not in ('avg', 'center'):
            return False
        if not isinstance(self.final_pointnet, PointNet) or len(self.knnlayer.layers) != 2 or len(self.final_pointnet.layers) != 2:
            return False
        k1, k2 = self.knnlayer.layers
        f1, f2 = self.final_pointnet.layers
        if k1.conv.in_channels != 3 + 384 or k2.conv.in_channels != k1.conv.out_channels or k1.conv.out_channels % 16 != 0 \
                or f1.conv.in_channels != 3 + k2.conv.out_channels or k2.conv.out_channels % 16 != 0 or f2.conv.in_channels != f1.conv.out_channels:
            return False
        return all(l._p16_ok() for l in (k1, k2, f1, f2))

    def _node_stage(self, xp, prep, B, M):
        K, G = prep["K"], prep["G"]
        k1, k2 = self.knnlayer.layers
        f1, f2 = self.final_pointnet.layers
        dev = xp.device
        C1 = k1.conv.out_channels
        z = _ops.pointmlp_h3p(xp, k1._packed_p16(lambda: k1._weight2d().detach()[:, 3:], "feat"), _ops.const_vec(C1, 1.0, dev),
                              _ops.const_vec(C1, 0.0, dev), False, C1, out="p16", tag="flat")
        s1, t1 = k1._eval_affine()
        h1 = _ops.knn_stage_input(prep, z, k1._lead_cols(3), s1, t1, k1.activation == 'relu')
        center, cp = prep["center"], prep["center_p16"]
        s2, t2 = k2._eval_affine()
        knn = _ops.pointmlp_h3p_gmax(h1, k2._packed_p16(), s2, t2, k2.activation == 'relu', k2.conv.out_channels, K, G, B * M, out="p16", Lout=xp.L)
        s3, t3 = f1._eval_affine()
        h3 = _ops.pointmlp_h3p(knn, f1._packed_p16(lambda: torch.cat((f1._weight2d().detach()[:, 3:], f1._weight2d().detach()[:, :3]), dim=1), "rot3"),
                               s3, t3, f1.activation == 'relu', f1.conv.out_channels, x2=cp, out="p16", tag="flat")
        s4, t4 = f2._eval_affine()
        feature = _ops.pointmlp_h3p_gmax(h3, f2._packed_p16(), s4, t4, f2.activation == 'relu', f2.conv.out_channels, M, 128 // M, B, out="f32")
        self.knn_center_1 = center
        self.__dict__["_stage"] = dict(knn_p16=knn, h3_p16=h3, B=B, M=M)
        self.__dict__["_knn_feature_1"] = None
        self.__dict__["_final_pn_out"] = None
        return feature

    def _forward_guarded(self, x, sn, node, node_knn_I, is_train, epoch):
        can_rerun = not (torch.is_grad_enabled() or self.training)
        return _ops.run_guarded(lambda: self._forward(x, sn, node, node_knn_I, is_train, epoch), x.device, can_rerun)

    def _forward(self, x, sn, node, node_knn_I, is_train=False, epoch=None):
        opt = self.opt
        M = node.size()[2]
        xd = x.detach().float().contiguous()
        sb = self.som_builder
        sb.node = node.detach().float().contiguous()
        use_sn = bool(opt.surface_normal)
        snd = sn.detach().float().contiguous() if use_sn else None
        fused_pool = (use_sn and _ops.FUSE_POOL and not getattr(self, 'want_first_pn_out', False)
                      and not torch.is_grad_enabled() and self.first_pointnet._fusable_eval(xd)
                      and int(opt.k) * xd.shape[2] * 384 * 4 < 4e9)
        stage = fused_pool and _ops.POINTMLP_PRECISION == "h3" and self._node_stage_ok(xd.shape[0], M, node_knn_I)
        knn = (node_knn_I.contiguous(), int(opt.som_k), opt.som_k_type == 'avg') if stage else None
        fast = sb.assign_sort(xd, snd, opt.k, knn=knn) if fused_pool else None
        if fast is not None:
            a, g = fast
        elif fused_pool:
            a = sb.assign(xd, opt.k)
            g = _ops.som_sort_group(xd, snd, a)
        else:
            a, g = None, None
        if fused_pool:
            sb.node = g["som_node"]
            self.som_node = sb.node
            self._lazy = dict(a=a, x=xd, sn=snd, mask=None, min_idx=None, centers=None, x_decentered=None)
            self._first_pn_out = None
            wstream, affine = self.first_pointnet._fused_state()
            self.__dict__["_stage"] = None
            if stage:
                prep = g.get("knn_prep")
                if prep is None:
                    prep = _ops.knn_stage_prepare(self.som_node, knn[0], knn[1], knn[2])
                self.first_pn_out_masked_max, xp = _ops.pointresnet_fused_pool(g, wstream, affine, M, want_p16=True)
                self.feature = self._node_stage(xp, prep, xd.shape[0], M)
                return self.feature
            pool = _ops.pointresnet_bf16_pool if _ops.POINTMLP_PRECISION == "bf16" else _ops.pointresnet_fused_pool
            self.first_pn_out_masked_max = pool(g, wstream, affine, M)
        else:
            self.__dict__["_stage"] = None
            train_pooled = torch.is_grad_enabled() and isinstance(self.first_pointnet, PointResNet) and getattr(self, "pooled_backward", True)
            per_point = self._wants_dense() if torch.is_grad_enabled() else bool(getattr(self, 'want_first_pn_out', False))
            sorted_pool = (train_pooled and use_sn and not per_point and a is None and self.first_pointnet.pooled_sorted_ok(xd, M)
                           and int(opt.k) * xd.shape[2] * 384 * 4 < 4e9)
            if sorted_pool:
                fast = sb.assign_sort(xd, snd, opt.k, deterministic=True) if _ops.TRAIN_ASSIGN_SORT else None
                if fast is not None:
                    a, g = fast
                else:
                    a = sb.assign(xd, opt.k)
                    g = _ops.som_sort_group(xd, snd, a)
                self._lazy = dict(a=a, x=xd, sn=snd, mask=None, min_idx=None, centers=None, x_decentered=None)
                pn_in = g["x_aug_sorted"]
            else:
                if a is None:
                    a = sb.assign(xd, opt.k)
                g = _ops.som_group(xd, snd, a, want_centers=per_point, want_decentered=(not use_sn) or per_point, want_augmented=use_sn)
                self._lazy = dict(a=a, x=xd, sn=snd, mask=None, min_idx=None,
                                  centers=g["centers"], x_decentered=g["x_decentered"])
                pn_in = g["x_augmented"] if use_sn else g["x_decentered"]
            sb.node = g["som_node"]
            self.som_node = sb.node
            row_max = g["row_max"]

            pooled = None
            if sorted_pool:
                pooled = self.first_pointnet.forward_pooled(pn_in, g["ids_sorted"], row_max, M, epoch, need_dense=False, pos0=g["pos0"])
            elif train_pooled:
                pooled = self.first_pointnet.forward_pooled(pn_in, a.min_idx_i32, row_max, M, epoch,
                                                            need_dense=per_point or not _ops.POOLED_TRAIN_EPILOGUE)
            if pooled is not None:
                self.first_pn_out, self.first_pn_out_masked_max, _ = pooled
                if self._first_pn_out is None:
                    self._lazy["not_materialised"] = True
            else:
                self.first_pn_out = self.first_pointnet(pn_in, epoch)
                if self._first_pn_out is None:
                    self._lazy["first_p16"] = self.first_pointnet.last_p16
                    _, self.first_pn_out_masked_max = _ops.index_max_gather_p16(self.first_pointnet.last_p16, a.min_idx_i32, M, row_max)
                elif torch.is_grad_enabled() and self.first_pn_out.requires_grad:
                    gather_index = _ops.index_max(self.first_pn_out.detach(), a.min_idx_i32, M).long()
                    self.first_pn_out_masked_max = self.first_pn_out.gather(
                        dim=2, index=gather_index * row_max.unsqueeze(1).long())
                else:
                    _, self.first_pn_out_masked_max = _ops.index_max_gather(self.first_pn_out, a.min_idx_i32, M, row_max)

        if opt.som_k >= 2:
            self.knn_center_1, self.knn_feature_1 = self.knnlayer(self.som_node, self.first_pn_out_masked_max,
                                                                  node_knn_I, opt.som_k, opt.som_k_type, epoch)
            lead, feat = self.knn_center_1, self.knn_feature_1
        else:
            lead, feat = self.som_node, self.first_pn_out_masked_max
        forward_cat = getattr(self.final_pointnet, 'forward_cat', None)
        self.final_pn_out = (forward_cat(lead, feat, epoch) if forward_cat is not None
                             else self.final_pointnet(torch.cat((lead, feat), dim=1), epoch))
        if torch.is_grad_enabled() and self.final_pn_out.requires_grad:
            self.feature = _ops.lastdim_max_autograd(self.final_pn_out)
        else:
            self.feature = _ops.lastdim_max(self.final_pn_out.contiguous())
        if self.feature.dtype != torch.float32:
            self.feature = self.feature.float()
        return self.feature


class Classifier(_PlainAttrs, nn.Module):

    def __init__(self, opt):
        super().__init__()
        self.opt = opt
        self.feature_num = opt.feature_num
        kw = _bn_kwargs(opt)
        self.fc1 = MyLinear(self.feature_num, 512, activation=opt.activation, normalization=opt.normalization, **kw)
        self.fc2 = MyLinear(512, 256, activation=opt.activation, normalization=opt.normalization, **kw)
        self.fc3 = MyLinear(256, opt.classes, activation=None, normalization=None)
        self.dropout1 = nn.Dropout(p=opt.dropout)
        self.dropout2 = nn.Dropout(p=opt.dropout)

    @_head_inference
    def forward(self, feature, epoch=None):
        h = self.fc1(feature, epoch)
        if self.opt.dropout > 0.1:
            h = self.dropout1(h)
        self.fc2_out = self.fc2(h, epoch)
        if self.opt.dropout > 0.1:
            self.fc2_out = self.dropout2(self.fc2_out)
        return self.fc3(self.fc2_out, epoch)


class Segmenter(_PlainAttrs, nn.Module):

    def __init__(self, opt):
        super().__init__()
        _DENSE_HEADS.add(self)
        self.opt = opt
        self.feature_num = opt.feature_num
        c = 3 + 3 + 3 + 16 + 384 + 384 + self.feature_num * 2
        if opt.surface_normal:
            c += 3
        if opt.som_k >= 2:
# ... 254 lines not shown
```

### so-net_amd/sonet_hip/_lib.py

```python
import ctypes
import os

import torch

_HERE = os.path.dirname(os.path.abspath(__file__))
LIB_PATH = os.path.join(os.path.dirname(_HERE), "lib", "libsonet_hip.so")
VARIANTS_PATH = os.path.join(os.path.dirname(_HERE), "lib", "libsonet_hip_variants.so")
if os.environ.get("SONET_HIP_LIB"):
    LIB_PATH = os.environ["SONET_HIP_LIB"]

_vp = ctypes.c_void_p
_i = ctypes.c_int

SIGNATURES = {
    "sonet_abi_version": [],
    "sonet_build_arch": [],
    "sonet_last_error": [],
    "sonet_check_device": [],
    "sonet_range_log_set": [_vp],
    "sonet_pooled_wgrad_f32": [_vp, _vp, _vp, _i, _i, _i, _i, _i, _vp, _vp],
    "sonet_bn_running_update_f32": [_vp, _vp, _vp, _vp, ctypes.c_float, ctypes.c_float, _i, _vp],
    "sonet_knn_prepare_f32": [_vp, _vp, _i, _i, _i, _i, _vp, _vp, _vp, _vp],
    "sonet_pointmlp_h3_gather_f32": [_vp, _i, _i, _vp, _vp, _i, _vp, _vp, _vp, _i, _vp, _i, _i, _i, _vp],
    "sonet_planes_max_f32": [_vp, _vp, ctypes.c_longlong, _i, _i, _vp],
    "sonet_diag_mfma_f16_rate": [_i, _i, _vp, _vp, _vp],
    "sonet_index_max_f32": [_vp, _vp, _vp, _i, _i, _i, _i, _vp],
    "sonet_index_max_bf16": [_vp, _vp, _vp, _i, _i, _i, _i, _vp],
    "sonet_index_max_gather_f32": [_vp, _vp, _vp, _vp, _vp, _i, _i, _i, _i, _vp],
    "sonet_som_assign_f32": [_vp, _vp, _i, _i, _i, _i, _vp, _vp, _vp, _vp, _vp],
    "sonet_som_train_f32": [_vp, _vp, _i, _vp, _vp, _i, _i, _i, _i, _vp, _vp],
    "sonet_assemble_batch_f32": [_vp, ctypes.c_longlong, _vp, _i, _vp, _vp, _i, _i, _i, _i, _i, ctypes.c_longlong, ctypes.c_longlong,
                                 _vp, _vp, _vp, _vp, _vp, _vp, _vp, _vp, _vp, _vp],
    "sonet_som_assign_sort_ws_size": [_i, _i, _i, _i],
    "sonet_pointmlp_bf16_pool": [_vp, _i, _vp, _i, _vp, _vp, _vp, _i, _vp, _vp, _vp, _vp, _i, _i, _i, _i, _vp],
    "sonet_pointmlp_bf16_pool_xaff": [_vp, _i, _vp, _i, _vp, _vp, _vp, _i, _vp, _vp, _vp, _vp, _i, _i, _i, _i, _vp, _vp, _vp, _vp, _i, _vp],
    "sonet_pointmlp_h3_segpool_ws_size": [_i, _i, _i],
    "sonet_pointmlp_h3_segpool_f32": [_vp, _i, _vp, _i, _vp, _vp, _vp, _i, _vp, _vp, _vp, _i, _vp, _vp, _vp, _i, _i, _i, _vp, _vp, _vp, _vp, _i, _vp],
    "sonet_pointmlp_h3_stats_xaff_f32": [_vp, _i, _vp, _i, _vp, _vp, _vp, _i, _vp, _i, _i, _i, _vp, _vp, _vp, _vp, _vp, _vp, _vp, _i, _vp],
    "sonet_pointmlp_x3_bnb_f32": [_vp, _vp, _i, _vp, _vp, _vp, _vp, _vp, _vp, _vp, _vp, _i, _vp, _vp, _i, _i, _i, _vp, _vp, _vp, _i, _vp, _vp, _vp],
    "sonet_pointmlp_x3_bnb_acc_f32": [_vp, _vp, _i, _vp, _vp, _vp, _vp, _vp, _vp, _vp, _vp, _i, _vp, _vp, _vp, _i, _i, _i, _vp],
    "sonet_wgrad_x3_xaff_f32": [_vp, _vp, _vp, _vp, _i, _i, _i, _i, _vp, _vp, _i, _vp],
    "sonet_pooled_wgrad_xaff_f32": [_vp, _vp, _vp, _i, _i, _i, _i, _i, _vp, _vp, _vp, _i, _vp],
    "sonet_pack_multi": [_vp, _i, _i, _vp],
    "sonet_pack_multi_kc": [_i, _i],
    "sonet_bn_rider_set": [_vp, _vp, ctypes.c_float, ctypes.c_float, ctypes.c_float, _vp, _vp, _vp, _vp, _vp],
    "sonet_som_assign_sort_f32": [_vp, _vp, _vp, _i, _i, _i, _i, _vp, _vp, _vp, _vp, _vp, _vp, _vp, _vp, _vp, _vp, _vp, _vp],
    "sonet_som_assign_sort_det_f32": [_vp, _vp, _vp, _i, _i, _i, _i, _vp, _vp, _vp, _vp, _vp, _vp, _vp, _vp, _vp, _vp, _vp, _vp],
    "sonet_som_assign_sort_knn_f32": [_vp, _vp, _vp, _i, _i, _i, _i, _vp, _vp, _vp, _vp, _vp, _vp, _vp, _vp, _vp, _vp, _vp,
                                      _vp, _i, _i, _i, _vp, _vp, _vp, _vp],
    "sonet_som_group_f32": [_vp, _vp, _vp, _vp, _vp, _i, _i, _i, _i, _vp, _vp, _vp, _vp, _vp, _vp],
    "sonet_som_mask_i32": [_vp, _vp, _i, _i, _i, _vp],
    "sonet_node_gather_f32": [_vp, _vp, _vp, _i, _i, _i, _i, _vp],
    "sonet_knn_self_f32": [_vp, _vp, _i, _i, _i, _vp],
    "sonet_knn_group_f32": [_vp, _vp, _vp, _i, _i, _i, _i, _i, _vp, _vp, _vp],
    "sonet_lastdim_max_f32": [_vp, _vp, ctypes.c_longlong, _i, _vp],
    "sonet_knn_gather_f32": [_vp, _vp, _vp, _i, _i, _i, _i, _vp],
    "sonet_pointmlp_pack_size": [_i, _i],
    "sonet_pointmlp_pack_f32": [_vp, _vp, _i, _i, _vp],
    "sonet_pointmlp_f32": [_vp, _i, _vp, _i, _vp, _vp, _vp, _i, _vp, _i, _i, _i, _vp],
    "sonet_pointmlp_bf16_pack_size": [_i, _i],
    "sonet_pointmlp_bf16_pack": [_vp, _vp, _i, _i, _vp],
    "sonet_pointmlp_bf16": [_vp, _i, _vp, _i, _vp, _vp, _vp, _i, _vp, _i, _i, _i, _vp],
    "sonet_pointmlp_bf16_acc": [_vp, _i, _vp, _i, _vp, _vp, _vp, _i, _vp, _vp, _i, _i, _i, _vp],
    "sonet_pointmlp_bf16_bnb": [_vp, _vp, _i, _vp, _vp, _vp, _vp, _vp, _vp, _vp, _vp, _i, _vp, _vp, _vp, _i, _i, _i, _vp],
    "sonet_pointmlp_bf16_gather": [_vp, _i, _i, _vp, _vp, _i, _vp, _vp, _vp, _i, _vp, _i, _i, _i, _vp],
    "sonet_index_max_gather_bf16": [_vp, _vp, _vp, _vp, _vp, _i, _i, _i, _i, _vp],
    "sonet_index_max_gather_p16": [_vp, _vp, _vp, _vp, _vp, _i, _i, _i, _i, _vp],
    "sonet_node_gather_lead_affine_act_f32": [_vp, _vp, _vp, _vp, _vp, _vp, _i, _vp, _i, _i, _i, _i, _i, _vp],
    "sonet_node_gather_lead_affine_act_bf16": [_vp, _vp, _vp, _vp, _vp, _vp, _i, _vp, _i, _i, _i, _i, _i, _vp],
    "sonet_pointmlp_stats_ws_size": [_i, _i, _i],
    "sonet_pointmlp_h3_stats_f32": [_vp, _i, _vp, _i, _vp, _vp, _vp, _i, _vp, _i, _i, _i, _vp, _vp, _vp, _vp],
    "sonet_pointmlp_x3_stats_f32": [_vp, _i, _vp, _i, _vp, _vp, _vp, _i, _vp, _i, _i, _i, _vp, _vp, _vp, _vp],
    "sonet_pointmlp_bf16_stats_ws_size": [_i, _i, _i],
    "sonet_pointmlp_bf16_stats": [_vp, _i, _vp, _i, _vp, _vp, _vp, _i, _vp, _i, _i, _i, _vp, _vp, _vp, _vp],
    "sonet_pointmlp_bf16_stats_xaff": [_vp, _i, _vp, _i, _vp, _vp, _vp, _i, _vp, _i, _i, _i, _vp, _vp, _vp, _vp, _vp, _vp, _vp, _i, _vp],
    "sonet_pointmlp_h3_nodeadd_f32": [_vp, _i, _vp, _i, _vp, _vp, _vp, _i, _vp, _i, _i, _i, _vp, _vp, _i, _vp],
    "sonet_wgrad_x3_ws_size": [_i, _i, _i, _i],
    "sonet_wgrad_x3_f32": [_vp, _vp, _vp, _vp, _i, _i, _i, _i, _vp],
    "sonet_wgrad_bf16_ws_size": [_i, _i, _i, _i],
    "sonet_wgrad_bf16": [_vp, _vp, _vp, _vp, _i, _i, _i, _i, _vp],
    "sonet_wgrad_bf16_xaff": [_vp, _vp, _vp, _vp, _i, _i, _i, _i, _vp, _vp, _i, _vp],
    "sonet_pointmlp_x3_pack_size": [_i, _i],
    "sonet_pointmlp_x3_pack": [_vp, _vp, _i, _i, _vp],
    "sonet_pointmlp_x3_f32": [_vp, _i, _vp, _i, _vp, _vp, _vp, _i, _vp, _i, _i, _i, _vp],
    "sonet_pointmlp_h3_pack": [_vp, _vp, _i, _i, _vp],
    "sonet_pointmlp_h3_f32": [_vp, _i, _vp, _i, _vp, _vp, _vp, _i, _vp, _i, _i, _i, _vp],
    "sonet_lastdim_argmax_f32": [_vp, _vp, _vp, ctypes.c_longlong, _i, _vp],
    "sonet_lastdim_argmax_bf16": [_vp, _vp, _vp, ctypes.c_longlong, _i, _vp],
    "sonet_lastdim_max_bwd_f32": [_vp, _vp, _vp, ctypes.c_longlong, _i, _vp],
    "sonet_lastdim_max_bwd_bf16": [_vp, _vp, _vp, ctypes.c_longlong, _i, _vp],
    "sonet_knn_gather_bwd_ws_size": [_i, _i, _i],
    "sonet_knn_gather_bwd_f32": [_vp, _vp, _vp, _vp, _i, _i, _i, _i, _vp],
    "sonet_knn_gather_bwd_bf16": [_vp, _vp, _vp, _vp, _i, _i, _i, _i, _vp],
    "sonet_node_gather_bwd_ws_size": [_i, _i, _i],
    "sonet_node_gather_bwd_f32": [_vp, _vp, _vp, _vp, _i, _i, _i, _i, _vp],
    "sonet_node_gather_bwd_bf16": [_vp, _vp, _vp, _vp, _i, _i, _i, _i, _vp],
    "sonet_p16_size": [_i, _i, _i],
    "sonet_p16_from_f32": [_vp, _vp, _i, _i, _i, _vp, _vp, _i, _vp],
    "sonet_p16_to_f32": [_vp, _vp, _i, _i, _i, _vp],
    "sonet_pointmlp_h3p_pack_size": [_i, _i],
    "sonet_pointmlp_h3p_pack": [_vp, _vp, _i, _i, _vp],
    "sonet_pointmlp_h3p_stats_ws_size": [_i, _i, _i],
    "sonet_pointmlp_h3p": [_vp, _i, _i, _vp, _vp, _i, _vp, _vp, _vp, _i, _vp, _vp, _i, _i, _i, _vp, _vp, _i, _vp, _vp, _vp, _vp],
    "sonet_pointresnet_bf16_pack_size": [],
    "sonet_pointresnet_bf16_pack": [_vp, _vp, _vp, _vp, _i, _vp, _vp],
    "sonet_pointresnet_bf16": [_vp, _i, _vp, _vp, _vp, _i, _i, _vp],
    "sonet_pointresnet_bf16_pool_ws_size": [_i, _i, _i],
    "sonet_pointresnet_bf16_pool": [_vp, _i, _vp, _vp, _vp, _vp, _vp, _vp, _vp, _vp, _i, _i, _i, _vp],
    "sonet_pointresnet_pack_size": [],
    "sonet_pointresnet_pack": [_vp, _vp, _vp, _vp, _i, _vp, _vp],
    "sonet_pointresnet_fused_f32": [_vp, _i, _vp, _vp, _vp, _i, _i, _vp],
    "sonet_pointresnet_fused_p16_f32": [_vp, _i, _vp, _vp, _vp, _vp, _i, _i, _vp],
    "sonet_pointresnet_pool_ws_size": [_i, _i, _i],
    "sonet_pointresnet_fused_pool_f32": [_vp, _i, _vp, _vp, _vp, _vp, _vp, _vp, _vp, _vp, _i, _i, _i, _vp],
    "sonet_pointresnet_fused_pool_p16_f32": [_vp, _i, _vp, _vp, _vp, _vp, _vp, _vp, _vp, _vp, _vp, _i, _i, _i, _vp],
    "sonet_knn_stage_columns": [_i, _i, _i],
    "sonet_knn_stage_prepare_f32": [_vp, _vp, _i, _i, _i, _i, _i, _vp, _vp, _vp, _vp],
    "sonet_knn_stage_input_p16": [_vp, _vp, _vp, _vp, _vp, _i, _i, _i, _i, _i, _vp, _vp],
    "sonet_pointmlp_h3p_gmax": [_vp, _i, _vp, _i, _vp, _vp, _vp, _i, _i, _i, _i, _i, _i, _i, _vp, _vp, _vp],
    "sonet_node_stage_columns": [_i, _i],
    "sonet_p16_flat_to_bcm_f32": [_vp, _vp, _i, _i, _i, _vp],
    "sonet_som_sort_group_f32": [_vp, _vp, _vp, _vp, _vp, _i, _i, _i, _i, _vp, _vp, _vp, _vp, _vp, _vp, _vp, _vp],
    "sonet_pointwise_bwd_stats_f32": [_vp, _vp, _vp, _vp, _i, _i, _i, _i, _vp, _vp],
    "sonet_pointwise_bwd_apply_f32": [_vp, _vp, _vp, _vp, _i, _vp, _vp, _vp, _vp, _i, _i, _i, _vp],
    "sonet_node_add_affine_act_f32": [_vp, _vp, _vp, _vp, _vp, _i, _i, _i, _i, _i, _vp],
    "sonet_linear_act_f32": [_vp, _vp, _vp, _vp, _i, _vp, _i, _i, _i, _vp],
    "sonet_pooled_dgrad_ws_size": [_i, _i, _i, _i],
    "sonet_pooled_wgrad_xbf16": [_vp, _vp, _vp, _i, _i, _i, _i, _i, _vp, _vp],
    "sonet_pooled_wgrad_xaff_xbf16": [_vp, _vp, _vp, _i, _i, _i, _i, _i, _vp, _vp, _vp, _i, _vp],
    "sonet_pooled_dgrad_obf16": [_vp, _vp, _vp, _i, _i, _i, _i, _i, _i, _vp, _vp, _vp, _vp],
    "sonet_pooled_dgrad_f32": [_vp, _vp, _vp, _i, _i, _i, _i, _i, _i, _vp, _vp, _vp, _vp],
    "sonet_pooled_dgrad_mfma_bf16": [_vp, _vp, _vp, _i, _i, _i, _i, _i, _i, _vp, _vp, _vp, _vp],
    "sonet_bn_fwd_coeffs_f32": [_vp, _vp, _vp, _vp, ctypes.c_float, _i, _vp, _vp, _vp, _vp],
    "sonet_bn_bwd_coeffs_f32": [_vp, _vp, _vp, _vp, ctypes.c_double, _i, _vp, _vp, _vp, _vp, _vp, _vp],
    "sonet_channel_affine_act_out_f32": [_vp, _vp, _vp, _i, _vp, _i, _i, _i, _vp],
    "sonet_chunk_mean_f32": [_vp, _vp, ctypes.c_longlong, _i, _i, _vp],
    "sonet_pointmlp_x3_pack_strided": [_vp, ctypes.c_longlong, ctypes.c_longlong, _vp, _i, _i, _i, _vp],
    "sonet_pointmlp_h3_pack_strided": [_vp, ctypes.c_longlong, ctypes.c_longlong, _vp, _i, _i, _i, _vp],
    "sonet_pointmlp_bf16_pack_strided": [_vp, ctypes.c_longlong, ctypes.c_longlong, _vp, _i, _i, _i, _vp],
    "sonet_adam_chunk": [],
    "sonet_fc_max_rows": [],
    "sonet_fc_bn_act_fwd_f32": [_vp, _vp, _vp, _vp, _vp, _vp, _vp, ctypes.c_float, ctypes.c_float, _i, _i, _i, _i, _vp, _vp, _vp, _vp],
    "sonet_fc_bn_act_bwd_f32": [_vp, _vp, _vp, _vp, _vp, _vp, _i, _i, _i, _i, _vp, _vp, _vp, _vp, _vp, _vp],
    "sonet_fc_dx_f32": [_vp, _vp, _i, _i, _i, _vp, _vp],
    "sonet_adam_multi_f32": [_vp, _vp, _vp, _vp, _vp, _vp, _i, ctypes.c_float, ctypes.c_float, ctypes.c_float, ctypes.c_float, ctypes.c_float, _vp],
    "sonet_channel_stats_f32": [_vp, _i, _i, _i, _vp, _vp, _vp, _vp],
    "sonet_channel_stats_bf16": [_vp, _i, _i, _i, _vp, _vp, _vp, _vp],
    "sonet_channel_affine_act_out_bf16": [_vp, _vp, _vp, _i, _vp, _i, _i, _i, _vp],
    "sonet_pointwise_bwd_stats_bf16": [_vp, _vp, _vp, _vp, _i, _i, _i, _i, _vp, _vp],
    "sonet_pointwise_bwd_apply_bf16": [_vp, _vp, _vp, _vp, _i, _vp, _vp, _vp, _vp, _i, _i, _i, _vp],
    "sonet_channel_affine_act_f32": [_vp, _vp, _vp, _i, _i, _i, _i, _vp],
    "sonet_chamfer_nn_f32": [_vp, _vp, _vp, _i, _i, _i, _vp],
}
_RESTYPES = {
    "sonet_build_arch": ctypes.c_char_p,
    "sonet_last_error": ctypes.c_char_p,
    "sonet_pointmlp_pack_size": ctypes.c_size_t,
    "sonet_pointmlp_stats_ws_size": ctypes.c_size_t,
    "sonet_pointmlp_h3_segpool_ws_size": ctypes.c_size_t,
    "sonet_pointmlp_bf16_stats_ws_size": ctypes.c_size_t,
    "sonet_wgrad_x3_ws_size": ctypes.c_size_t,
    "sonet_wgrad_bf16_ws_size": ctypes.c_size_t,
    "sonet_pointmlp_x3_pack_size": ctypes.c_size_t,
    "sonet_p16_size": ctypes.c_size_t,
    "sonet_knn_stage_columns": ctypes.c_size_t,
    "sonet_node_stage_columns": ctypes.c_size_t,
    "sonet_knn_gather_bwd_ws_size": ctypes.c_size_t,
    "sonet_node_gather_bwd_ws_size": ctypes.c_size_t,
    "sonet_pointmlp_h3p_pack_size": ctypes.c_size_t,
    "sonet_pointmlp_h3p_stats_ws_size": ctypes.c_size_t,
    "sonet_pointmlp_bf16_pack_size": ctypes.c_size_t,
    "sonet_pointresnet_pack_size": ctypes.c_size_t,
    "sonet_pointresnet_bf16_pack_size": ctypes.c_size_t,
    "sonet_pointresnet_bf16_pool_ws_size": ctypes.c_size_t,
    "sonet_pointresnet_pool_ws_size": ctypes.c_size_t,
    "sonet_pooled_dgrad_ws_size": ctypes.c_size_t,
    "sonet_pooled_dgrad_tail_ws_size": ctypes.c_size_t,
    "sonet_som_assign_sort_ws_size": ctypes.c_size_t,
    "sonet_chamfer_nn2_ws_size": ctypes.c_size_t,
}

VARIANT_SIGNATURES = {
    "sonet_chamfer_nn2_ws_size": [_i, _i, _i],
    "sonet_chamfer_nn2_f32": [_vp, _vp, _vp, _vp, _vp, _i, _i, _i, _vp],
    "sonet_pointmlp_h3_kmax_f32": [_vp, _i, _vp, _i, _vp, _vp, _vp, _i, _vp, _vp, _i, _i, _i, _i, _vp],
    "sonet_pooled_dgrad_tail_ws_size": [_i, _i, _i],
    "sonet_pooled_dgrad_tail_f32": [_vp, _vp, _vp, _i, _i, _i, _i, _i, _i, _vp, _vp, _vp, _vp, _vp, _vp, _vp, _vp, _i, _vp, _vp, _vp],
}

_lib = None


class SonetHipError(RuntimeError):
    pass


def load():
    global _lib
    if _lib is not None:
        return _lib
    if not os.path.exists(LIB_PATH):
        raise SonetHipError(
            "libsonet_hip.so is not built (%s).  Build it with `make -C so-net_amd/csrc` or "
            "`python -c 'import __graft_entry__ as g; g.build()'`.  There is no CPU fallback." % LIB_PATH)
    try:
        lib = ctypes.CDLL(LIB_PATH)
    except OSError as e:
        raise SonetHipError("cannot load %s: %s" % (LIB_PATH, e))
    for name, args in SIGNATURES.items():
        fn = getattr(lib, name)
        fn.argtypes = args
        fn.restype = _RESTYPES.get(name, ctypes.c_int)
    for name, args in VARIANT_SIGNATURES.items():
        fn = getattr(lib, name, None)
        if fn is not None:
            fn.argtypes = args
            fn.restype = _RESTYPES.get(name, ctypes.c_int)
    _lib = lib
    return lib


def last_error():
    return load().sonet_last_error().decode("utf-8", "replace")


def check(status, what=""):
    if status != 0:
        raise SonetHipError("%s failed (status %d): %s" % (what or "libsonet_hip", status, last_error()))


_device_ok = {}


def require_device(device):
    if device.index in _device_ok:
        return
    if not torch.cuda.is_available():
        raise SonetHipError("sonet_hip needs an MI355X (gfx950) GPU; torch.cuda.is_available() is False "
                            "and there is no CPU fallback")
    idx = device.index if device.index is not None else torch.cuda.current_device()
    ok = _device_ok.get(idx)
    if ok is None:
        with torch.cuda.device(idx):
            check(load().sonet_check_device(), "sonet_check_device")
        _device_ok[idx] = True


def stream_ptr():
    return ctypes.c_void_p(torch._C._cuda_getCurrentRawStream(torch._C._cuda_getDevice()))


class on_device:
    __slots__ = ("idx", "prev")

    def __init__(self, dev):
        self.idx = dev.index if dev.index is not None else -1

    def __enter__(self):
        self.prev = torch.cuda._exchange_device(self.idx)

    def __exit__(self, *exc):
        torch.cuda._maybe_exchange_device(self.prev)
        return False


def ptr(t):
    return ctypes.c_void_p(t.data_ptr()) if t is not None else None
```

### so-net_amd/sonet_hip/ops.py

```python
import numpy as np
import torch

from . import _lib
from ._lib import SonetHipError, check, ptr, stream_ptr
import functools as _functools
import threading as _threading

_tls = _threading.local()
_join_lock = _threading.Lock()


def _consumes_rider(fn):
    @_functools.wraps(fn)
    def wrapped(*a, **k):
        try:
            return fn(*a, **k)
        finally:
            _rider_done()
    return wrapped


_TIMING = None


# ... 551 lines not shown
def assemble_batch(src, offsets, nodes_src, idx, N, K, flags, seed, step, replay_idx=None, replay_draws=None, want_draws=False,
                   sizes=None):
    _chk(src, "src", torch.float32, 2)
    _chk(offsets, "offsets", torch.int64, 1)
    _chk(nodes_src, "nodes_src", torch.float32, 3)
    _chk(idx, "idx", torch.int64, 1)
    S, M = nodes_src.shape[0], nodes_src.shape[1]
    B, N, K, flags = idx.shape[0], int(N), int(K), int(flags)
    if src.shape[0] != 6 or nodes_src.shape[2] != 3 or offsets.shape[0] != S + 1:
        raise SonetHipError("src must be 6 x P, nodes_src S x M x 3 and offsets S+1, got %s, %s, %s"
                            % (tuple(src.shape), tuple(nodes_src.shape), tuple(offsets.shape)))
    if B < 1 or N < 1 or not 1 <= K <= min(M, BATCH_MAX_K):
        raise SonetHipError("need B >= 1, N >= 1 and 1 <= K <= min(M, %d), got B=%d N=%d K=%d M=%d" % (BATCH_MAX_K, B, N, K, M))
    if sizes is not None:
        ii, sizes = idx.cpu().numpy(), np.asarray(sizes)
        if ii.min() < 0 or ii.max() >= S:
            raise SonetHipError("idx out of range [0, %d): min %d max %d" % (S, ii.min(), ii.max()))
        smallest = int(sizes[ii].min())
        if not flags & BATCH_SHAPENET and smallest < N:
            raise SonetHipError("N=%d > n_s=%d points of a cloud in the batch (modelnet / shrec sample without replacement)" % (N, smallest))
    dev = _same_device(src, offsets, nodes_src, idx, replay_idx, replay_draws)
    D = batch_draw_size(N, M)
    if replay_idx is not None:
        _chk(replay_idx, "replay_idx", torch.int64)
        if tuple(replay_idx.shape) != (B, N):
            raise SonetHipError("replay_idx must be B x N = %s, got %s" % ((B, N), tuple(replay_idx.shape)))
    if replay_draws is not None:
        _chk(replay_draws, "replay_draws", torch.float64)
        if tuple(replay_draws.shape) != (B, D):
            raise SonetHipError("replay_draws must be B x D = %s, got %s" % ((B, D), tuple(replay_draws.shape)))
    f32 = dict(dtype=torch.float32, device=dev)
    r = dict(pc=torch.empty((B, 3, N), **f32), sn=torch.empty((B, 3, N), **f32), node=torch.empty((B, 3, M), **f32),
             chosen=torch.empty((B, N), dtype=torch.int64, device=dev), knn_I=torch.empty((B, M, K), dtype=torch.int64, device=dev),
             bad=torch.empty((B,), dtype=torch.int32, device=dev))
    if want_draws:
        r["draws"] = torch.zeros((B, D), dtype=torch.float64, device=dev)
    with _lib.on_device(dev), _timed("assemble_batch"):
        check(_lib.load().sonet_assemble_batch_f32(
            ptr(src), src.shape[1], ptr(offsets), S, ptr(nodes_src), ptr(idx), B, N, M, K, flags, _i64(seed), _i64(step), ptr(replay_idx) if replay_idx is not None else None,
            ptr(replay_draws) if replay_draws is not None else None, ptr(r["draws"]) if want_draws else None,
            ptr(r["pc"]), ptr(r["sn"]), ptr(r["node"]), ptr(r["chosen"]), ptr(r["knn_I"]), ptr(r["bad"]), stream_ptr()),
            "sonet_assemble_batch_f32")
    return r


def knn_group(coord, feat, knn_I, center_avg):
    _chk(coord, "coord", torch.float32, 3)
    _chk(feat, "feat", torch.float32, 3)
    _chk(knn_I, "knn_I", torch.int64, 3)
    dev = _same_device(coord, feat, knn_I)
    B, C, M = feat.shape
    K = knn_I.shape[2]
    center = torch.empty((B, 3, M), dtype=torch.float32, device=dev)
    out = torch.empty((B, 3 + C, M, K), dtype=torch.float32, device=dev)
    with _lib.on_device(dev), _timed("knn_group"):
        check(_lib.load().sonet_knn_group_f32(ptr(coord), ptr(feat), ptr(knn_I), B, C, M, K, int(bool(center_avg)), ptr(center), ptr(out),
                                              stream_ptr()), "sonet_knn_group_f32")
    return center, out


def lastdim_max(x):
    if x.dtype == torch.bfloat16:
        x = x.float()
    if not x.is_contiguous() or x.dtype != torch.float32:
        raise SonetHipError("lastdim_max needs a contiguous float32 tensor")
    dev = _same_device(x)
    K = x.shape[-1]
    out = torch.empty(x.shape[:-1], dtype=torch.float32, device=dev)
    if out.numel() == 0:
        return out
    with _lib.on_device(dev), _timed("lastdim_max"):
        check(_lib.load().sonet_lastdim_max_f32(ptr(x), ptr(out), out.numel(), K, stream_ptr()), "sonet_lastdim_max_f32")
    return out


def knn_gather(x, knn_I):
    _chk(x, "som_node", torch.float32, 3)
    _chk(knn_I, "som_node_knn_I", torch.int64, 3)
    B, C, M = x.shape
    if knn_I.shape[0] != B or knn_I.shape[1] != M:
        raise SonetHipError("knn_I must be B x M x K, got %s for x %s" % (tuple(knn_I.shape), tuple(x.shape)))
    K = knn_I.shape[2]
    dev = _same_device(x, knn_I)
    out = torch.empty((B, C, M, K), dtype=torch.float32, device=dev)
    with _lib.on_device(dev), _timed("knn_gather"):
        check(_lib.load().sonet_knn_gather_f32(ptr(x), ptr(knn_I), ptr(out), B, C, M, K, stream_ptr()), "sonet_knn_gather_f32")
    return out


def knn_gather_bwd(g, knn_I, M):
    if g.dtype not in (torch.float32, torch.bfloat16):
        raise SonetHipError("knn_gather_bwd: f32 or bf16 gradient")
    _chk(g, "g", g.dtype, 4)
    _chk(knn_I, "som_node_knn_I", torch.int64, 3)
    B, C, Mq, K = g.shape
    if tuple(knn_I.shape) != (B, Mq, K) or Mq != M:
        raise SonetHipError("knn_gather_bwd: knn_I must be B x M x K with the M of the gathered tensor")
    dev = _same_device(g, knn_I)
    lib = _lib.load()
    gx = torch.empty((B, C, M), dtype=torch.float32, device=dev)
    ws = torch.empty((lib.sonet_knn_gather_bwd_ws_size(B, M, K),), dtype=torch.uint8, device=dev)
    fn = lib.sonet_knn_gather_bwd_bf16 if g.dtype == torch.bfloat16 else lib.sonet_knn_gather_bwd_f32
    with _lib.on_device(dev), _timed("knn_gather_bwd"):
        check(fn(ptr(g), ptr(knn_I), ptr(gx), ptr(ws), B, C, M, K, stream_ptr()), "sonet_knn_gather_bwd")
    return gx


class _LastDimMax(torch.autograd.Function):

    @staticmethod
    def forward(ctx, x):
        xc = x.contiguous()
        K = xc.shape[-1]
        rows = xc.numel() // K
        out = torch.empty(xc.shape[:-1], dtype=xc.dtype, device=xc.device)
        idx = torch.empty(xc.shape[:-1], dtype=torch.int32, device=xc.device)
        lib = _lib.load()
        fn = lib.sonet_lastdim_argmax_bf16 if xc.dtype == torch.bfloat16 else lib.sonet_lastdim_argmax_f32
        with _lib.on_device(xc.device), _timed("lastdim_argmax"):
            check(fn(ptr(xc), ptr(out), ptr(idx), rows, K, stream_ptr()), "sonet_lastdim_argmax")
        ctx.save_for_backward(idx)
        ctx.K = K
        return out

    @staticmethod
    def backward(ctx, g):
        (idx,) = ctx.saved_tensors
        gc = g.contiguous()
        gx = torch.empty(tuple(gc.shape) + (ctx.K,), dtype=gc.dtype, device=gc.device)
        lib = _lib.load()
        fn = lib.sonet_lastdim_max_bwd_bf16 if gc.dtype == torch.bfloat16 else lib.sonet_lastdim_max_bwd_f32
        with _lib.on_device(gc.device), _timed("lastdim_max_bwd"):
            check(fn(ptr(gc), ptr(idx), ptr(gx), gc.numel(), ctx.K, stream_ptr()), "sonet_lastdim_max_bwd")
        return gx


def lastdim_max_autograd(x):
    if not x.is_cuda or x.dtype not in (torch.float32, torch.bfloat16) or x.numel() == 0:
        return torch.max(x, dim=-1)[0]
    return _LastDimMax.apply(x)


import os as _os

POINTMLP_PRECISION = _os.environ.get("SONET_POINTMLP_PRECISION", "h3")


FUSE_POINTRESNET = _os.environ.get("SONET_FUSE_POINTRESNET", "1") != "0"
FUSE_POOL = _os.environ.get("SONET_FUSE_POOL", "1") != "0"
GATHER_NODE_STAGE = _os.environ.get("SONET_GATHER_NODE_STAGE", "1") != "0"
NODE_LINEAR_SPLIT = _os.environ.get("SONET_NODE_LINEAR_SPLIT", "1") != "0"
P16_CHAINS = _os.environ.get("SONET_P16_CHAINS", "1") != "0"
NODE_STAGE_P16 = _os.environ.get("SONET_NODE_STAGE_P16", "1") != "0"
POOLED_TRAIN_EPILOGUE = _os.environ.get("SONET_POOLED_TRAIN_EPILOGUE", "1") != "0"
H3_SEGPOOL = _os.environ.get("SONET_H3_SEGPOOL", "1") != "0"
H3_NORM_ON_LOAD = _os.environ.get("SONET_H3_NORM_ON_LOAD", "1") != "0"
TRAIN_ASSIGN_SORT = _os.environ.get("SONET_TRAIN_ASSIGN_SORT", "1") != "0"
WGRAD_KERNEL = _os.environ.get("SONET_WGRAD_KERNEL", "1") != "0"


RANGE_GUARD = _os.environ.get("SONET_RANGE_GUARD", "1") != "0"
_RANGE_SLOTS = 32
_B_2047, _B_65504, _B_XLOW, _B_WLOW, _B_WLOW32 = 0x44FFE000, 0x477FE000, 0x3C800000, 0x3B800000, 0x3E000000
_range_logs = {}
_range_active = None
_range_ptr_set = False


def _bits_to_float(u):
    import struct
    return struct.unpack("<f", struct.pack("<I", int(u) & 0xFFFFFFFF))[0]


class range_scope:

    def __init__(self, device, private=False):
        self.device = torch.device(device)
        self.names = []
        self.enabled = RANGE_GUARD and self.device.type == "cuda"
        self.log = None
        self._prev = None
        self._own = torch.zeros((_RANGE_SLOTS * 8,), dtype=torch.int32, device=self.device) if (private and self.enabled) else None

    def __enter__(self):
        global _range_active
        self._prev = _range_active
        if self.enabled:
            idx = self.device.index if self.device.index is not None else torch.cuda.current_device()
            log = self._own if self._own is not None else _range_logs.get(idx)
            if log is None:
                log = torch.zeros((_RANGE_SLOTS * 8,), dtype=torch.int32, device=self.device)
                _range_logs[idx] = log
            else:
                log.zero_()
            self.log = log
            _range_active = self
        return self

    def __exit__(self, *exc):
        global _range_active
        _range_active = self._prev
        _range_unset()
        return False

    def _slot(self, name):
        i = min(len(self.names), _RANGE_SLOTS - 1)
        self.names.append(name)
        return self.log.data_ptr() + i * 32

    def violations(self):
        if not self.enabled or not self.names:
            return []
        w = self.log.cpu().view(_RANGE_SLOTS, 8).tolist()
        shared = {}
        out = []
        for n, name in enumerate(self.names):
            i = min(n, _RANGE_SLOTS - 1)
            if i in shared:
                continue
            shared[i] = True
            x, wt, hid = (v & 0xFFFFFFFF for v in w[i][:3])
            low_ok = n < _RANGE_SLOTS - 1
            if x > _B_2047:
                out.append((name, "max |x| = %g exceeds 2047" % _bits_to_float(x)))
            elif low_ok and 0 < x < _B_XLOW:
                out.append((name, "max |x| = %g is below 2^-6 (fp16 residuals go subnormal)" % _bits_to_float(x)))
            if name.startswith("pointresnet_fused"):
                if wt > _B_65504:
                    out.append((name, "max |w| = %g exceeds %g" % (_bits_to_float(wt) / 32.0, 65504.0 / 32.0)))
                elif low_ok and 0 < wt < _B_WLOW32:
                    out.append((name, "max |w| = %g is below 2^-8" % (_bits_to_float(wt) / 32.0)))
            elif name.startswith("pointmlph3p"):
                if wt > _B_2047:
                    out.append((name, "max |w| = %g exceeds 2047" % _bits_to_float(wt)))
                elif low_ok and 0 < wt < _B_WLOW:
                    out.append((name, "max |w| = %g is below 2^-8" % _bits_to_float(wt)))
            elif wt > _B_65504:
                out.append((name, "max |w| = %g exceeds 65504" % _bits_to_float(wt)))
            elif low_ok and 0 < wt < _B_WLOW:
                out.append((name, "max |w| = %g is below 2^-8" % _bits_to_float(wt)))
            if hid > _B_2047:
                out.append((name, "a hidden activation reaches %g > 2047" % _bits_to_float(hid)))
        return out


_range_warned = False
_range_pending = []


def range_warn(bad):
    global _range_warned
    if not _range_warned:
        import warnings
        warnings.warn("sonet_hip: fp16-split (h3) operand range left by %d launch(es), e.g. %s: %s -- recomputing in the "
                      "range-safe x3 arithmetic (SONET_POINTMLP_PRECISION=x3 selects it from the start)"
                      % (len(bad), bad[0][0], bad[0][1]), RuntimeWarning, stacklevel=3)
        _range_warned = True


def _range_defer(scope):
    if not scope.enabled or not scope.names or torch.cuda.is_current_stream_capturing():
        return
    host = torch.empty((_RANGE_SLOTS * 8,), dtype=torch.int32, pin_memory=True)
    host.copy_(scope.log, non_blocking=True)
    ev = torch.cuda.Event()
    ev.record()
    _range_pending.append((ev, host, list(scope.names)))


range_scope.defer = _range_defer


def range_deferred_check():
    global POINTMLP_PRECISION
    while _range_pending and _range_pending[0][0].query():
        _, host, names = _range_pending.pop(0)
        probe = range_scope.__new__(range_scope)
        probe.enabled, probe.names, probe.log = True, names, host
        bad = probe.violations()
        if bad:
            range_warn(bad)
            POINTMLP_PRECISION = "x3"
            _range_pending.clear()
            return bad
    return []


def run_guarded(call, device, can_rerun):
    device = torch.device(device)
    if POINTMLP_PRECISION != "h3" or not RANGE_GUARD or device.type != "cuda" or _range_active is not None:
        return call()
    if not can_rerun:
        range_deferred_check()
        if POINTMLP_PRECISION != "h3":
            return call()
        with range_scope(device) as rs:
            out = call()
        rs.defer()
        return out
    with range_scope(device) as rs:
        out = call()
    if torch.cuda.is_current_stream_capturing():
        return out
    bad = rs.violations()
    if bad:
        range_warn(bad)
# ... 633 lines not shown
        with _lib.on_device(p.device), _timed("p16_to_f32"):
            check(_lib.load().sonet_p16_to_f32(ptr(p.data), ptr(x), p.B, p.C, p.L, stream_ptr()), "sonet_p16_to_f32")
    return x


def pointmlp_h3p_pack(weight2d):
    _chk(weight2d, "weight", torch.float32, 2)
    dev = _same_device(weight2d)
    Cout, Cin = weight2d.shape
    lib = _lib.load()
    with _lib.on_device(dev):
        wp = torch.empty((lib.sonet_pointmlp_h3p_pack_size(Cin, Cout) // 4,), dtype=torch.int32, device=dev)
        check(lib.sonet_pointmlp_h3p_pack(ptr(weight2d), ptr(wp), Cin, Cout, stream_ptr()), "sonet_pointmlp_h3p_pack")
    return wp


@_consumes_rider
def pointmlp_h3p(x1, wp, scale, shift, relu, Cout, x2=None, out="f32", gidx=None, z=None, zidx=None, stats=False, tag=None):
    if not isinstance(x1, P16) or (x2 is not None and not isinstance(x2, P16)):
        raise SonetHipError("pointmlp_h3p: P16 inputs (ops.p16_from_f32)")
    if wp.dtype != torch.int32:
        raise SonetHipError("pointmlp_h3p: an h3p pack (ops.pointmlp_h3p_pack)")
    B, C1, L1 = x1.shape
    L = L1
    if gidx is not None:
        _chk(gidx, "gidx", torch.int32, 2)
        if gidx.shape[0] != B:
            raise SonetHipError("pointmlp_h3p: gidx must have B rows")
        L = gidx.shape[1]
    C2 = 0
    if x2 is not None:
        if x2.B != B or x2.L != L:
            raise SonetHipError("x2 must be B x C2 x L")
        C2 = x2.C
        if C1 % 16 != 0:
            raise SonetHipError("pointmlp_h3p: with a second input C1 must be a multiple of 16")
    _chk(scale, "scale", torch.float32, 1)
    _chk(shift, "shift", torch.float32, 1)
    if (z is None) != (zidx is None):
        raise SonetHipError("pointmlp_h3p: z and zidx come together")
    ZM = 0
    if z is not None:
        _chk(z, "z", torch.float32, 3)
        _chk(zidx, "zidx", torch.int32, 2)
        if tuple(z.shape[:2]) != (B, Cout) or tuple(zidx.shape) != (B, L):
            raise SonetHipError("pointmlp_h3p: z must be B x Cout x M and zidx B x L")
        ZM = z.shape[2]
    if out not in ("f32", "p16", "both") or (stats and out != "f32"):
        raise SonetHipError("pointmlp_h3p: out is 'f32', 'p16' or 'both' (statistics: 'f32')")
    dev = _same_device(x1.data, x2.data if x2 is not None else None, wp, scale, shift, gidx, z, zidx)
    lib = _lib.load()
    cin_pack = (C1 + C2) if C2 else C1
    if wp.numel() * 4 != lib.sonet_pointmlp_h3p_pack_size(cin_pack, Cout):
        raise SonetHipError("packed weight has %d bytes, expected %d for Cin=%d Cout=%d"
                            % (wp.numel() * 4, lib.sonet_pointmlp_h3p_pack_size(cin_pack, Cout), cin_pack, Cout))
    y = torch.empty((B, Cout, L), dtype=torch.float32, device=dev) if out in ("f32", "both") else None
    yp = p16_empty(B, Cout, L, dev) if out in ("p16", "both") else None
    mean = var = ws = None
    if stats:
        mean = torch.empty((Cout,), dtype=torch.float32, device=dev)
        var = torch.empty((Cout,), dtype=torch.float32, device=dev)
        ws = torch.empty((lib.sonet_pointmlp_h3p_stats_ws_size(B, Cout, L),), dtype=torch.uint8, device=dev)
    if B * L * Cout != 0:
        name = "pointmlph3p%s_%dx%d_L%d" % ("_nodeadd" if z is not None else "_stats" if stats else ("_" + tag) if tag else "", C1 + C2, Cout, L)
        _range_arm(name)
        with _lib.on_device(dev), _timed(name):
            check(lib.sonet_pointmlp_h3p(ptr(x1.data), C1, L1, ptr(gidx), ptr(x2.data) if x2 is not None else None, C2, ptr(wp), ptr(scale), ptr(shift),
                                         int(bool(relu)), ptr(y), ptr(yp.data) if yp is not None else None, B, Cout, L, ptr(z), ptr(zidx), ZM,
                                         ptr(ws), ptr(mean), ptr(var), stream_ptr()), "sonet_pointmlp_h3p")
    if stats:
        return y, mean, var
    return y if out == "f32" else yp if out == "p16" else (y, yp)


def node_stage_columns(B, M):
    return (B * M + 127) // 128 * 128


def p16_flat(C, L, nvalid, device):
    if nvalid == L:
        return p16_empty(1, C, L, device)
    n = _lib.load().sonet_p16_size(1, C, L)
    return P16(torch.zeros((n,), dtype=torch.uint8, device=device), 1, C, L)


def pointmlp_h3p_gmax(x1, wp, scale, shift, relu, Cout, GK, G, ngout, x2=None, out="p16", Lout=None):
    if not isinstance(x1, P16) or (x2 is not None and not isinstance(x2, P16)):
        raise SonetHipError("pointmlp_h3p_gmax: P16 inputs")
    if wp.dtype != torch.int32:
        raise SonetHipError("pointmlp_h3p_gmax: an h3p pack (ops.pointmlp_h3p_pack)")
    if x1.B != 1 or (x2 is not None and (x2.B != 1 or x2.L != x1.L)):
        raise SonetHipError("pointmlp_h3p_gmax: one flat cloud (B == 1), x2 with the columns of x1")
    if out not in ("p16", "f32"):
        raise SonetHipError("pointmlp_h3p_gmax: out is 'p16' or 'f32'")
    C1, L = x1.C, x1.L
    C2 = x2.C if x2 is not None else 0
    _chk(scale, "scale", torch.float32, 1)
    _chk(shift, "shift", torch.float32, 1)
    dev = _same_device(x1.data, x2.data if x2 is not None else None, wp, scale, shift)
    lib = _lib.load()
    if wp.numel() * 4 != lib.sonet_pointmlp_h3p_pack_size(C1 + C2, Cout):
        raise SonetHipError("packed weight has %d bytes, expected %d for Cin=%d Cout=%d"
                            % (wp.numel() * 4, lib.sonet_pointmlp_h3p_pack_size(C1 + C2, Cout), C1 + C2, Cout))
    Lout = int(ngout if Lout is None else Lout)
    y = torch.empty((ngout, Cout), dtype=torch.float32, device=dev) if out == "f32" else None
    yp = p16_flat(Cout, Lout, ngout, dev) if out == "p16" else None
    name = "pointmlph3p_gmax%d_%dx%d_L%d" % (GK, C1 + C2, Cout, int(ngout) * int(GK))
    _range_arm(name)
    with _lib.on_device(dev), _timed(name):
        check(lib.sonet_pointmlp_h3p_gmax(ptr(x1.data), C1, ptr(x2.data) if x2 is not None else None, C2, ptr(wp), ptr(scale), ptr(shift),
                                          int(bool(relu)), Cout, L, int(GK), int(G), int(ngout), Lout, ptr(y), ptr(yp.data) if yp is not None else None,
                                          stream_ptr()), "sonet_pointmlp_h3p_gmax")
    return y if out == "f32" else yp


def knn_stage_prepare(coord, knn_I, K, center_avg):
    _chk(coord, "coord", torch.float32, 3)
    _chk(knn_I, "knn_I", torch.int64, 3)
    B, three, M = coord.shape
    KI = knn_I.shape[2]
    if three != 3 or tuple(knn_I.shape[:2]) != (B, M) or KI < K or not 1 <= K <= 128:
        raise SonetHipError("knn_stage_prepare: coord B x 3 x M, knn_I B x M x (>= K), 1 <= K <= 128")
    dev = _same_device(coord, knn_I)
    lib = _lib.load()
    Lm = node_stage_columns(B, M)
    Lp = int(lib.sonet_knn_stage_columns(B, M, int(K)))
    center = torch.empty((B, 3, M), dtype=torch.float32, device=dev)
    cp = p16_flat(3, Lm, B * M, dev)
    rec = torch.empty((Lp, 4), dtype=torch.int32, device=dev)
    _range_arm("knn_stage_prepare")
    with _lib.on_device(dev), _timed("knn_stage_prepare"):
        check(lib.sonet_knn_stage_prepare_f32(ptr(coord), ptr(knn_I), KI, int(bool(center_avg)), B, M, int(K), ptr(center), ptr(cp.data), ptr(rec),
                                              stream_ptr()), "sonet_knn_stage_prepare_f32")
    return dict(center=center, center_p16=cp, rec=rec, B=B, M=M, K=int(K), G=min(16, 128 // int(K)), Lp=Lp)


def knn_stage_input(prep, z, wl, scale, shift, relu):
    if not isinstance(z, P16) or z.B != 1 or z.L != node_stage_columns(prep["B"], prep["M"]):
        raise SonetHipError("knn_stage_input: z is a P16 1 x C x Lm activation")
    _chk(wl, "wl", torch.float32, 2)
    _chk(scale, "scale", torch.float32, 1)
    _chk(shift, "shift", torch.float32, 1)
    C = z.C
    if tuple(wl.shape) != (C, 3) or scale.numel() != C or shift.numel() != C:
        raise SonetHipError("knn_stage_input: wl C x 3, scale / shift C")
    dev = _same_device(prep["rec"], z.data, wl, scale, shift)
    h1 = p16_empty(1, C, prep["Lp"], dev)
    name = "knn_stage_input_%dx%d" % (C, prep["B"] * prep["M"] * prep["K"])
    _range_arm(name)
    with _lib.on_device(dev), _timed(name):
        check(_lib.load().sonet_knn_stage_input_p16(ptr(prep["rec"]), ptr(z.data), ptr(wl), ptr(scale), ptr(shift), int(bool(relu)),
                                                    prep["B"], prep["M"], prep["K"], C, ptr(h1.data), stream_ptr()), "sonet_knn_stage_input_p16")
    return h1


def p16_flat_to_bcm(p, B, M):
    if p.B != 1 or p.L != node_stage_columns(B, M):
        raise SonetHipError("p16_flat_to_bcm: a 1 x C x (B M) activation")
    x = torch.empty((B, p.C, M), dtype=torch.float32, device=p.device)
    with _lib.on_device(p.device), _timed("p16_flat_to_bcm"):
        check(_lib.load().sonet_p16_flat_to_bcm_f32(ptr(p.data), ptr(x), B, p.C, M, stream_ptr()), "sonet_p16_flat_to_bcm_f32")
    return x


def pointresnet_pack(w1, w2, w3, w4):
    for i, w in enumerate((w1, w2, w3, w4)):
        _chk(w, "w%d" % (i + 1), torch.float32, 2)
    if (w1.shape[0], tuple(w2.shape), tuple(w3.shape), tuple(w4.shape)) != (64, (128, 64), (256, 128), (384, 320)) or w1.shape[1] > 16:
        raise SonetHipError("pointresnet_fused supports Cin0<=16 -> 64 -> 128 -> 256 -> [320] -> 384 only")
    dev = _same_device(w1, w2, w3, w4)
    lib = _lib.load()
    ws = torch.empty((lib.sonet_pointresnet_pack_size(),), dtype=torch.uint8, device=dev)
    with _lib.on_device(dev):
        check(lib.sonet_pointresnet_pack(ptr(w1), ptr(w2), ptr(w3), ptr(w4), w1.shape[1], ptr(ws), stream_ptr()),
              "sonet_pointresnet_pack")
    return ws


def pointresnet_fused(x, wstream, affine, want_p16=False):
    _chk(x, "x", torch.float32, 3)
    _chk(affine, "affine", torch.float32, 2)
    if tuple(affine.shape) != (832, 2):
        raise SonetHipError("affine must be 832 x 2 (scale, shift)")
    dev = _same_device(x, wstream, affine)
    B, Cin0, L = x.shape
    only = want_p16 == "only"
    y = None if only else torch.empty((B, 384, L), dtype=torch.float32, device=dev)
    yp = p16_empty(B, 384, L, dev) if want_p16 else None
    if B * L == 0:
        return (y, yp) if want_p16 else y
    _range_arm("pointresnet_fused_L%d" % L)
    with _lib.on_device(dev), _timed("pointresnet_fused%s_L%d" % ("_p16only" if only else "_p16" if want_p16 else "", L)):
        if want_p16:
            check(_lib.load().sonet_pointresnet_fused_p16_f32(ptr(x), Cin0, ptr(wstream), ptr(affine), ptr(y), ptr(yp.data), B, L, stream_ptr()),
                  "sonet_pointresnet_fused_p16_f32")
        else:
            check(_lib.load().sonet_pointresnet_fused_f32(ptr(x), Cin0, ptr(wstream), ptr(affine), ptr(y), B, L, stream_ptr()),
                  "sonet_pointresnet_fused_f32")
    return (y, yp) if want_p16 else y


def pointresnet_fused_pool(sg, wstream, affine, M, want_p16=False):
    x_sorted = sg["x_aug_sorted"]
    _chk(x_sorted, "x_sorted", torch.float32, 3)
    _chk(affine, "affine", torch.float32, 2)
    dev = _same_device(x_sorted, wstream, affine, sg["ids_sorted"], sg["pos0"], sg["node_off"], sg["count"])
    B, Cin0, L = x_sorted.shape
    lib = _lib.load()
    ws = torch.empty((lib.sonet_pointresnet_pool_ws_size(B, L, int(M)),), dtype=torch.uint8, device=dev)
    out = torch.empty((B, 384, int(M)), dtype=torch.float32, device=dev)
    outp = p16_flat(384, node_stage_columns(B, int(M)), B * int(M), dev) if want_p16 else None
    _range_arm("pointresnet_fused_pool_L%d" % L)
    with _lib.on_device(dev), _timed("pointresnet_fused_pool_L%d" % L):
        if want_p16:
            check(lib.sonet_pointresnet_fused_pool_p16_f32(ptr(x_sorted), Cin0, ptr(wstream), ptr(affine), ptr(sg["ids_sorted"]), ptr(sg["pos0"]),
                                                           ptr(sg["node_off"]), ptr(sg["count"]), ptr(ws), ptr(out), ptr(outp.data), B, L, int(M),
                                                           stream_ptr()), "sonet_pointresnet_fused_pool_p16_f32")
        else:
            check(lib.sonet_pointresnet_fused_pool_f32(ptr(x_sorted), Cin0, ptr(wstream), ptr(affine), ptr(sg["ids_sorted"]), ptr(sg["pos0"]),
                                                       ptr(sg["node_off"]), ptr(sg["count"]), ptr(ws), ptr(out), B, L, int(M), stream_ptr()),
                  "sonet_pointresnet_fused_pool_f32")
    return (out, outp) if want_p16 else out


def pointresnet_bf16_pack(w1, w2, w3, w4):
    for i, w in enumerate((w1, w2, w3, w4)):
        _chk(w, "w%d" % (i + 1), torch.float32, 2)
    if (w1.shape[0], tuple(w2.shape), tuple(w3.shape), tuple(w4.shape)) != (64, (128, 64), (256, 128), (384, 320)) or w1.shape[1] > 16:
        raise SonetHipError("pointresnet_bf16 supports Cin0<=16 -> 64 -> 128 -> 256 -> [320] -> 384 only")
    dev = _same_device(w1, w2, w3, w4)
    lib = _lib.load()
    ws = torch.empty((lib.sonet_pointresnet_bf16_pack_size(),), dtype=torch.uint8, device=dev)
    with _lib.on_device(dev):
        check(lib.sonet_pointresnet_bf16_pack(ptr(w1), ptr(w2), ptr(w3), ptr(w4), w1.shape[1], ptr(ws), stream_ptr()),
              "sonet_pointresnet_bf16_pack")
    return ws


def pointresnet_bf16(x, wstream, affine):
    _chk(x, "x", torch.float32, 3)
    _chk(affine, "affine", torch.float32, 2)
    if tuple(affine.shape) != (832, 2):
        raise SonetHipError("affine must be 832 x 2 (scale, shift)")
    dev = _same_device(x, wstream, affine)
    B, Cin0, L = x.shape
    y = torch.empty((B, 384, L), dtype=torch.bfloat16, device=dev)
    if y.numel() == 0:
        return y
    with _lib.on_device(dev), _timed("pointresnet_bf16_L%d" % L):
        check(_lib.load().sonet_pointresnet_bf16(ptr(x), Cin0, ptr(wstream), ptr(affine), ptr(y), B, L, stream_ptr()),
              "sonet_pointresnet_bf16")
    return y


def pointresnet_bf16_pool(sg, wstream, affine, M):
    x_sorted = sg["x_aug_sorted"]
    _chk(x_sorted, "x_sorted", torch.float32, 3)
    _chk(affine, "affine", torch.float32, 2)
    dev = _same_device(x_sorted, wstream, affine, sg["ids_sorted"], sg["pos0"], sg["node_off"], sg["count"])
    B, Cin0, L = x_sorted.shape
    lib = _lib.load()
    ws = torch.empty((lib.sonet_pointresnet_bf16_pool_ws_size(B, L, int(M)),), dtype=torch.uint8, device=dev)
    out = torch.empty((B, 384, int(M)), dtype=torch.float32, device=dev)
    with _lib.on_device(dev), _timed("pointresnet_bf16_pool_L%d" % L):
        check(lib.sonet_pointresnet_bf16_pool(ptr(x_sorted), Cin0, ptr(wstream), ptr(affine), ptr(sg["ids_sorted"]), ptr(sg["pos0"]),
                                              ptr(sg["node_off"]), ptr(sg["count"]), ptr(ws), ptr(out), B, L, int(M), stream_ptr()),
              "sonet_pointresnet_bf16_pool")
    return out


@_consumes_rider
def channel_stats(y):
    _chk(y, "y", dim=3)
    if y.dtype not in (torch.float32, torch.bfloat16):
        raise SonetHipError("channel_stats: float32 or bfloat16, got %s" % y.dtype)
    dev = _same_device(y)
    B, C, L = y.shape
    ws = torch.empty((2 * C,), dtype=torch.float64, device=dev)
    mean = torch.empty((C,), dtype=torch.float32, device=dev)
    var = torch.empty((C,), dtype=torch.float32, device=dev)
    lib = _lib.load()
    fn = lib.sonet_channel_stats_f32 if y.dtype == torch.float32 else lib.sonet_channel_stats_bf16
    try:
        with _lib.on_device(dev), _timed("channel_stats" if y.dtype == torch.float32 else "channel_stats_bf16"):
            check(fn(ptr(y), B, C, L, ptr(ws), ptr(mean), ptr(var), stream_ptr()), "sonet_channel_stats")
    finally:
        _rider_done()
    return mean, var


def channel_affine_act_(y, scale, shift, relu):
    _chk(y, "y", torch.float32, 3)
    dev = _same_device(y, scale, shift)
    B, C, L = y.shape
    with _lib.on_device(dev), _timed("channel_affine_act"):
        check(_lib.load().sonet_channel_affine_act_f32(ptr(y), ptr(scale), ptr(shift), int(bool(relu)), B, C, L, stream_ptr()),
              "sonet_channel_affine_act_f32")
    return y


def channel_affine_act(x, scale, shift, relu):
    _chk(x, "x", dim=3)
    dev = _same_device(x, scale, shift)
    B, C, L = x.shape
    y = torch.empty_like(x)
    lib = _lib.load()
# ... 335 lines not shown
```

Baseline: 73210.

## Fuse kNN stage input formation into the group-max h3p GEMM kernel

Result: no change. 72810 (-0.5%).

```diff
diff --git a/include/sonet_hip.h b/include/sonet_hip.h
--- a/include/sonet_hip.h
+++ b/include/sonet_hip.h
@@ -136,6 +136,9 @@
                               int B, int M, int K, int C, void *h1_p16, sonet_stream_t stream);
 int sonet_pointmlp_h3p_gmax(const void *x1p, int C1, const void *x2p, int C2, const void *Wp, const float *scale, const float *shift,
                             int relu, int Cout, int L, int GK, int G, int ngout, int Lout, float *y, void *yp, sonet_stream_t stream);
+int sonet_pointmlp_h3p_gmax_knn(const void *rec, const void *z_p16, int C, const float *wl, const float *kscale, const float *kshift, int krelu,
+                                const void *Wp, const float *scale, const float *shift, int relu, int Cout, int B, int M, int K, int Lout, void *yp,
+                                sonet_stream_t stream);
 int sonet_p16_flat_to_bcm_f32(const void *p16, float *x, int B, int C, int M, sonet_stream_t stream);
 
 int sonet_lastdim_argmax_f32(const float *x, float *out, int32_t *idx, long long rows, int K, sonet_stream_t stream);
diff --git a/so-net_amd/csrc/common.hpp b/so-net_amd/csrc/common.hpp
--- a/so-net_amd/csrc/common.hpp
+++ b/so-net_amd/csrc/common.hpp
@@ -100,3 +100,34 @@
     m = __builtin_bit_cast(unsigned, __builtin_convertvector(R, sonet_h2_t));
 }
 static inline int knn_stage_groups(int K) { const int g = 128 / K; return g > 16 ? 16 : g; }
+
+typedef float knn_f2 __attribute__((ext_vector_type(2)));
+typedef _Float16 knn_h2 __attribute__((ext_vector_type(2)));
+__device__ __forceinline__ void knn_h1_pair(unsigned zh, unsigned zm, knn_f2 w0, knn_f2 w1, knn_f2 w2, knn_f2 sc, knn_f2 sh,
+                                            knn_f2 d0, knn_f2 d1, knn_f2 d2, bool valid, float lo, RangeAcc &xr, unsigned &hv, unsigned &mv)
+{
+    const knn_h2 zh2 = __builtin_bit_cast(knn_h2, zh), zm2 = __builtin_bit_cast(knn_h2, zm);
+    knn_f2 a = __builtin_convertvector(zh2, knn_f2) + __builtin_convertvector(zm2, knn_f2);
+    a = __builtin_elementwise_fma(w0, d0, a);
+    a = __builtin_elementwise_fma(w1, d1, a);
+    a = __builtin_elementwise_fma(w2, d2, a);
+    a = __builtin_elementwise_fma(a, sc, sh);
+    if (!valid) a = knn_f2{0.f, 0.f};
+    range_track(xr, a[0], a[1]);
+    const knn_f2 X = {__builtin_amdgcn_fmed3f(a[0], lo, 65504.f), __builtin_amdgcn_fmed3f(a[1], lo, 65504.f)};
+    const knn_h2 hp = __builtin_convertvector(X, knn_h2);
+    const knn_f2 R = X - __builtin_convertvector(hp, knn_f2);
+    hv = __builtin_bit_cast(unsigned, hp);
+    mv = __builtin_bit_cast(unsigned, __builtin_convertvector(R, knn_h2));
+}
+__device__ __forceinline__ unsigned knn_h1_range_bits(const RangeAcc &xr, bool relu) {
+    unsigned bits;
+    if (relu) {
+        const unsigned pos = xr.mp > 0 ? (unsigned)xr.mp : 0u, nan_neg = xr.mn > 0xFF800000u ? (xr.mn & 0x7FFFFFFFu) : 0u;
+        bits = pos > nan_neg ? pos : nan_neg;
+    } else {
+        bits = range_amax_bits(xr);
+    }
+    const unsigned wm = wave_umax(bits);
+    return wm > (5u << 23) ? wm - (5u << 23) : 0u;
+}
diff --git a/so-net_amd/csrc/node_stage.hip b/so-net_amd/csrc/node_stage.hip
--- a/so-net_amd/csrc/node_stage.hip
+++ b/so-net_amd/csrc/node_stage.hip
@@ -64,8 +64,7 @@
     }
 }
 
-typedef float ks_f2 __attribute__((ext_vector_type(2)));
-typedef _Float16 ks_h2 __attribute__((ext_vector_type(2)));
+typedef knn_f2 ks_f2;
 
 constexpr int KS_MAXG = 8;
 
@@ -129,19 +128,7 @@
                 const ks_f2 w0 = *reinterpret_cast<const ks_f2 *>(&coef[0][slot]), w1 = *reinterpret_cast<const ks_f2 *>(&coef[1][slot]),
                             w2 = *reinterpret_cast<const ks_f2 *>(&coef[2][slot]), sc = *reinterpret_cast<const ks_f2 *>(&coef[3][slot]),
                             sh = *reinterpret_cast<const ks_f2 *>(&coef[4][slot]);
-                const ks_h2 zh2 = __builtin_bit_cast(ks_h2, zh[q]), zm2 = __builtin_bit_cast(ks_h2, zm[q]);
-                ks_f2 a = __builtin_convertvector(zh2, ks_f2) + __builtin_convertvector(zm2, ks_f2);
-                a = __builtin_elementwise_fma(w0, d0, a);
-                a = __builtin_elementwise_fma(w1, d1, a);
-                a = __builtin_elementwise_fma(w2, d2, a);
-                a = __builtin_elementwise_fma(a, sc, sh);
-                if (!valid) a = ks_f2{0.f, 0.f};
-                range_track(xr, a[0], a[1]);
-                const ks_f2 X = {__builtin_amdgcn_fmed3f(a[0], lo, 65504.f), __builtin_amdgcn_fmed3f(a[1], lo, 65504.f)};
-                const ks_h2 hp = __builtin_convertvector(X, ks_h2);
-                const ks_f2 R = X - __builtin_convertvector(hp, ks_f2);
-                hv[q] = __builtin_bit_cast(unsigned, hp);
-                mv[q] = __builtin_bit_cast(unsigned, __builtin_convertvector(R, ks_h2));
+                knn_h1_pair(zh[q], zm[q], w0, w1, w2, sc, sh, d0, d1, d2, valid, lo, xr, hv[q], mv[q]);
             }
 #ifdef SONET_VARIANTS
             if ((abl & 1) && hv[0] != 0x12345u) { hq += 4 * Lp; continue; }
@@ -166,15 +153,7 @@
         }
     }
     if (rlog != nullptr) {
-        unsigned bits;
-        if (relu) {
-            const unsigned pos = xr.mp > 0 ? (unsigned)xr.mp : 0u, nan_neg = xr.mn > 0xFF800000u ? (xr.mn & 0x7FFFFFFFu) : 0u;
-            bits = pos > nan_neg ? pos : nan_neg;
-        } else {
-            bits = range_amax_bits(xr);
-        }
-        unsigned wm = wave_umax(bits);
-        wm = wm > (5u << 23) ? wm - (5u << 23) : 0u;
+        const unsigned wm = knn_h1_range_bits(xr, relu);
         if ((threadIdx.x & 63) == 0) wmax[threadIdx.x >> 6] = wm;
         __syncthreads();
         if (threadIdx.x == 0) {
diff --git a/so-net_amd/csrc/pointmlp_h3p.hip b/so-net_amd/csrc/pointmlp_h3p.hip
--- a/so-net_amd/csrc/pointmlp_h3p.hip
+++ b/so-net_amd/csrc/pointmlp_h3p.hip
@@ -145,6 +145,9 @@
     long long ngroups;
     int KC1, KC2, L1, L, Cout, CT, KC, KCr, KCP, ct_per_y, nslab, ncol, gpc, relu, ZM;
     int GK, G, ngout, Lout;
+    const int4 *krec;
+    const float *kwl, *ksc, *ksh;
+    int kC, krelu;
 };
 
 __device__ __forceinline__ i32x4_t make_rsrc(const void *base, unsigned bytes) {
@@ -188,6 +191,7 @@
     __builtin_amdgcn_sched_group_barrier(0x008, NC == 2 ? 3 : 2, 0);
 }
 
+constexpr int KNN_KC = 32;
 constexpr int GM_STRIDE = 136;
 __device__ __forceinline__ float nan_max(float m, float v) { return (v > m || v != v) ? v : m; }
 __device__ __forceinline__ void lds_barrier() { asm volatile("s_waitcnt lgkmcnt(0)\n\ts_barrier" ::: "memory"); }
@@ -196,7 +200,9 @@
 __global__ __launch_bounds__(P_THREADS, OCC) void pointmlp_h3p_kernel(const H3pArgs a)
 {
     static_assert(OUT >= 1 && OUT <= 3 && (EPI != 2 || (OUT & 1)), "output mode");
-    static_assert(EPI < 4 || (NC == 1 && ((EPI == 4 && OUT == 2) || (EPI == 5 && OUT == 1))), "group-max epilogues: 32-column waves, P16 (4) or f32 (5) out");
+    static_assert(EPI < 4 || (NC == 1 && (((EPI == 4 || EPI == 6) && OUT == 2) || (EPI == 5 && OUT == 1))),
+                  "group-max epilogues: 32-column waves, P16 (4, 6) or f32 (5) out");
+    constexpr bool GMAX_P16 = EPI == 4 || EPI == 6;
     static_assert(MT % 2 == 0 && (NC == 1 || NC == 2), "tile shape");
     constexpr int PB = (OCC >= 2 && NC == 2 && (EPI == 1 || EPI == 3)) ? 2 : 3, NB = 4, D = 3, NSLOT = D + 2;
     static_assert(D >= PB && PB >= 2, "the wait count below assumes the W request of a chunk is older than its X request");
@@ -212,6 +218,7 @@
         float2 red[EPI == 2 ? 4 : 1][EPI == 2 ? MT * 32 : 1];
         float zl[EPI == 1 ? MT * 32 : 1][EPI == 1 ? 64 : 1];
         float gm[EPI >= 4 ? 32 : 1][EPI >= 4 ? GM_STRIDE : 1];
+        __attribute__((aligned(16))) float kco[EPI == 6 ? KNN_KC : 1][2][40];
     };
     __shared__ __attribute__((aligned(16))) Lds lds;
 
@@ -232,6 +239,8 @@
     bool pv[NC];
     unsigned vo1[NC], vo2[NC], voy[NC], voyp[NC];
     int lcl[NC];
+    bool kvalid = true;
+    knn_f2 kd0 = {0.f, 0.f}, kd1 = kd0, kd2 = kd0;
 #pragma unroll
     for (int c = 0; c < NC; ++c) {
         const int l = l0 + 32 * c + j;
@@ -243,6 +252,14 @@
             const int src = a.gidx[(size_t)b * L + lcl[c]];
             vo1[c] = (unsigned)src < (unsigned)L1 ? (unsigned)(h * L1 + src) * 16u : OOB;
         }
+        if constexpr (EPI == 6) {
+            const int4 r = a.krec[lcl[c]];
+            vo1[c] = (unsigned)r.x < (unsigned)L1 ? (unsigned)(h * L1 + r.x) * 16u : OOB;
+            kvalid = r.x != -2;
+            kd0 = knn_f2{__int_as_float(r.y), __int_as_float(r.y)};
+            kd1 = knn_f2{__int_as_float(r.z), __int_as_float(r.z)};
+            kd2 = knn_f2{__int_as_float(r.w), __int_as_float(r.w)};
+        }
         voy[c] = pv[c] ? (unsigned)(4 * h * L + l) * 4u : OOB;
         voyp[c] = pv[c] ? (unsigned)(h * L + l) * 16u : OOB;
 #ifdef SONET_VARIANTS
@@ -329,6 +346,27 @@
     RangeAcc yr = {0, 0u};
     const float relu_thr = a.relu ? 0.f : -__builtin_inff();
     const float split_lo = a.relu ? 0.f : -2047.f;
+    RangeAcc kxr = {0, 0u};
+    const float klo = a.krelu ? 0.f : -65504.f;
+    auto knn_form = [&](u32x4 (&bb)[NBL], int kc) {
+        if constexpr (EPI == 6) {
+            const float *cf = &lds.kco[kc][h][0];
+            const bool v = kvalid && kc < a.KC1;
+            u32x4 hv, mv;
+#pragma unroll
+            for (int q = 0; q < 4; ++q) {
+                const knn_f2 w0 = *reinterpret_cast<const knn_f2 *>(cf + 2 * q), w1 = *reinterpret_cast<const knn_f2 *>(cf + 8 + 2 * q),
+                             w2 = *reinterpret_cast<const knn_f2 *>(cf + 16 + 2 * q), sc = *reinterpret_cast<const knn_f2 *>(cf + 24 + 2 * q),
+                             sh = *reinterpret_cast<const knn_f2 *>(cf + 32 + 2 * q);
+                unsigned hq, mq;
+                knn_h1_pair(bb[0][q], bb[1][q], w0, w1, w2, sc, sh, kd0, kd1, kd2, v, klo, kxr, hq, mq);
+                hv[q] = hq;
+                mv[q] = mq;
+            }
+            bb[0] = hv;
+            bb[1] = mv;
+        }
+    };
     int zm[NC];
     bool zok[NC];
     unsigned zvo[NC], zla[NC];
@@ -367,7 +405,7 @@
                 }
                 lds_barrier();
                 const int t = (int)threadIdx.x;
-                if constexpr (EPI == 4) {
+                if constexpr (GMAX_P16) {
                     const int p = t & 3, u = t >> 2;
                     const int g = u % a.G, qh = u / a.G;
                     if (qh < 4) {
@@ -559,7 +597,21 @@
         t[0] = scv;
         t[16] = shv;
     }
+    if constexpr (EPI == 6) {
+        for (int t = (int)threadIdx.x; t < KNN_KC * 16; t += P_THREADS) {
+            const int kc = t >> 4, hh = (t >> 3) & 1, e = t & 7;
+            const int c = kc * 16 + p16_channel(hh, e);
+            const bool in = c < a.kC;
+            float *k = &lds.kco[kc][hh][e];
+            k[0] = in ? 32.f * a.kwl[c * 3 + 0] : 0.f;
+            k[8] = in ? 32.f * a.kwl[c * 3 + 1] : 0.f;
+            k[16] = in ? 32.f * a.kwl[c * 3 + 2] : 0.f;
+            k[24] = in ? a.ksc[c] : 0.f;
+            k[32] = in ? 32.f * a.ksh[c] : 0.f;
+        }
+    }
     __syncthreads();
+    knn_form(bq[0], 0);
 #ifdef SONET_VARIANTS
     pt_pro = __builtin_readcyclecounter() - pt0;
 #endif
@@ -567,6 +619,7 @@
     int kcb = PB;
     int kcd = (1 + D) % KCr, passd = (1 + D) / KCr;
     int slot = 0;
+    int kcx = 0;
     if (kcb >= KCr) kcb -= KCr;
 
 #define H3P_BODY(I)                                                                                                   \
@@ -583,6 +636,7 @@
                 else wait_barrier<KWAIT>(bq[((I) + 1) & 3][0], bq[((I) + 1) & 3][1], bq[((I) + 1) & 3][2], bq[((I) + 1) & 3][3]); \
                 dma(passd, kcd, slotd);                                                                               \
                 read_a(Aq[cur ^ 1], slot1, 0);                                                                        \
+                knn_form(bq[((I) + 1) & 3], kcx + 1 < KCr ? kcx + 1 : 0);                                             \
             } else {                                                                                                  \
                 read_a(Aq[cur ^ 1], slot, p + 1);                                                                     \
             }                                                                                                         \
@@ -592,6 +646,7 @@
         }                                                                                                             \
         slot = slot1;                                                                                                 \
         kcb = kcb + 1 < KCr ? kcb + 1 : 0;                                                                            \
+        kcx = kcx + 1 < KCr ? kcx + 1 : 0;                                                                            \
         if (kcd + 1 < KCr) kcd += 1; else { kcd = 0; passd += 1; }                                                    \
     }
 
@@ -643,6 +698,7 @@
             if constexpr (OUT == 2) bits = bits > (5u << 23) ? bits - (5u << 23) : 0u;
             range_publish(a.rlog + 2, bits, lane);
         }
+        if constexpr (EPI == 6) range_publish(a.rlog + 2, knn_h1_range_bits(kxr, a.krelu != 0), lane);
         if (ct_begin == 0 && wg_col == 0 && threadIdx.x == 0)
             atomicMax(a.rlog + 1, reinterpret_cast<const unsigned *>(wp + (size_t)a.CT * a.KCP * 2048u)[0]);
     }
@@ -729,6 +785,7 @@
     else if (epi == 0 && out == 3) H3P_GO(0, 3);
     else if (epi == 4 && out == 2) { if constexpr (NC == 1) H3P_GO(4, 2); else return 1; }
     else if (epi == 5 && out == 1) { if constexpr (NC == 1) H3P_GO(5, 1); else return 1; }
+    else if (epi == 6 && out == 2) { if constexpr (NC == 1 && OCC == 2) H3P_GO(6, 2); else return 1; }
     else return 1;
 #undef H3P_GO
     return 0;
@@ -738,9 +795,9 @@
 static int h3p_launch(const char *what, const void *x1p, int C1, int L1, const int32_t *gidx, const void *x2p, int C2, const void *Wp,
                       const float *scale, const float *shift, int relu, float *y, void *yp, int B, int Cout, int L,
                       const float *zadd, const int32_t *zidx, int ZM, void *stats_ws, float *mean, float *var,
-                      int GK, int G, int ngout, int Lout, sonet_stream_t stream)
-{
-    if (!gidx) L1 = L;
+                      int GK, int G, int ngout, int Lout, sonet_stream_t stream, const H3pArgs *knn = nullptr)
+{
+    if (!gidx && !knn) L1 = L;
     SONET_REQUIRE(x1p && Wp && scale && shift && (y || yp), "%s: NULL pointer", what);
     SONET_REQUIRE(B > 0 && C1 > 0 && C2 >= 0 && Cout > 0 && L > 0 && L1 > 0, "%s: non-positive size", what);
     SONET_REQUIRE((C2 == 0) == (x2p == nullptr), "%s: x2 and C2 disagree", what);
@@ -768,6 +825,7 @@
     int nslab = 1;
     for (int d = 1; d <= groups; ++d)
         if (groups % d == 0 && (d <= 4 || cols < 131072 || CT / nslab > (zadd ? 16 : 32))) nslab = d;
+    if (knn) nslab = groups;
 #ifdef SONET_VARIANTS
     if (const char *e = sonet::knob("SONET_H3P_NSLAB")) {
         const int want = atoi(e);
@@ -789,8 +847,10 @@
     a.KC1 = KC1; a.KC2 = KC2; a.L1 = L1; a.L = L; a.Cout = Cout; a.CT = CT; a.KC = KC; a.KCr = KCr; a.KCP = KCP; a.ct_per_y = CT / nslab;
     a.nslab = nslab; a.ncol = (int)ncol; a.gpc = gpc; a.relu = relu; a.ZM = ZM;
     a.GK = GK; a.G = G; a.ngout = ngout; a.Lout = Lout;
+    a.krec = knn ? knn->krec : nullptr; a.kwl = knn ? knn->kwl : nullptr; a.ksc = knn ? knn->ksc : nullptr; a.ksh = knn ? knn->ksh : nullptr;
+    a.kC = knn ? knn->kC : 0; a.krelu = knn ? knn->krelu : 0;
     hipStream_t st = sonet::as_stream(stream);
-    const int epi = GK ? (yp ? 4 : 5)
+    const int epi = GK ? (yp ? (knn ? 6 : 4) : 5)
                        : stats_ws ? 2 : zadd ? ((ZM == 64 && gpc % 4 == 0 && CT / nslab <= 16 && Cout % 64 == 0) ? 1 : 3) : 0;
     const unsigned g = (unsigned)nwg;
     const int out = (y ? 1 : 0) | (yp ? 2 : 0);
@@ -830,3 +890,20 @@
     return h3p_launch(what, x1p, C1, L, nullptr, x2p, C2, Wp, scale, shift, relu, y, yp, 1, Cout, L, nullptr, nullptr, 0, nullptr, nullptr, nullptr,
                       GK, G, ngout, Lout, stream);
 }
+
+extern "C" int sonet_pointmlp_h3p_gmax_knn(const void *rec, const void *z_p16, int C, const float *wl, const float *kscale, const float *kshift,
+                                           int krelu, const void *Wp, const float *scale, const float *shift, int relu, int Cout, int B, int M, int K,
+                                           int Lout, void *yp, sonet_stream_t stream)
+{
+    const char *what = "sonet_pointmlp_h3p_gmax_knn";
+    SONET_REQUIRE(rec && z_p16 && wl && kscale && kshift && yp, "%s: NULL pointer", what);
+    SONET_REQUIRE(B > 0 && M > 0 && C > 0 && K >= 1 && K <= 128, "%s: bad size B=%d M=%d C=%d K=%d", what, B, M, C, K);
+    SONET_REQUIRE((long long)Lout >= (long long)B * M, "%s: Lout=%d below B M", what, Lout);
+    if (C > 16 * KNN_KC) return sonet::fail(SONET_ERR_UNSUPPORTED, "%s: C=%d above %d (the coefficient table)", what, C, 16 * KNN_KC);
+    const long long Lp = (long long)sonet_knn_stage_columns(B, M, K), Lm = (long long)sonet_node_stage_columns(B, M);
+    if (Lp > 0x7FFFFFFFll || (long long)B * M > 0x7FFFFFFFll) return sonet::fail(SONET_ERR_UNSUPPORTED, "%s: too many columns", what);
+    H3pArgs k;
+    k.krec = reinterpret_cast<const int4 *>(rec); k.kwl = wl; k.ksc = kscale; k.ksh = kshift; k.kC = C; k.krelu = krelu ? 1 : 0;
+    return h3p_launch(what, z_p16, C, (int)Lm, nullptr, nullptr, 0, Wp, scale, shift, relu, nullptr, yp, 1, Cout, (int)Lp, nullptr, nullptr, 0,
+                      nullptr, nullptr, nullptr, K, knn_stage_groups(K), B * M, Lout, stream, &k);
+}
diff --git a/so-net_amd/models/networks.py b/so-net_amd/models/networks.py
--- a/so-net_amd/models/networks.py
+++ b/so-net_amd/models/networks.py
@@ -225,10 +225,15 @@
         z = _ops.pointmlp_h3p(xp, k1._packed_p16(lambda: k1._weight2d().detach()[:, 3:], "feat"), _ops.const_vec(C1, 1.0, dev),
                               _ops.const_vec(C1, 0.0, dev), False, C1, out="p16", tag="flat")
         s1, t1 = k1._eval_affine()
-        h1 = _ops.knn_stage_input(prep, z, k1._lead_cols(3), s1, t1, k1.activation == 'relu')
         center, cp = prep["center"], prep["center_p16"]
         s2, t2 = k2._eval_affine()
-        knn = _ops.pointmlp_h3p_gmax(h1, k2._packed_p16(), s2, t2, k2.activation == 'relu', k2.conv.out_channels, K, G, B * M, out="p16", Lout=xp.L)
+        if _ops.KNN_GMAX_FUSED and C1 <= _ops.KNN_GMAX_FUSED_MAX_C:
+            knn = _ops.knn_gmax_fused(prep, z, k1._lead_cols(3), s1, t1, k1.activation == 'relu', k2._packed_p16(), s2, t2,
+                                      k2.activation == 'relu', k2.conv.out_channels, xp.L)
+        else:
+            h1 = _ops.knn_stage_input(prep, z, k1._lead_cols(3), s1, t1, k1.activation == 'relu')
+            knn = _ops.pointmlp_h3p_gmax(h1, k2._packed_p16(), s2, t2, k2.activation == 'relu', k2.conv.out_channels, K, G, B * M, out="p16",
+                                         Lout=xp.L)
         s3, t3 = f1._eval_affine()
         h3 = _ops.pointmlp_h3p(knn, f1._packed_p16(lambda: torch.cat((f1._weight2d().detach()[:, 3:], f1._weight2d().detach()[:, :3]), dim=1), "rot3"),
                                s3, t3, f1.activation == 'relu', f1.conv.out_channels, x2=cp, out="p16", tag="flat")
diff --git a/so-net_amd/sonet_hip/_lib.py b/so-net_amd/sonet_hip/_lib.py
--- a/so-net_amd/sonet_hip/_lib.py
+++ b/so-net_amd/sonet_hip/_lib.py
@@ -118,6 +118,7 @@
     "sonet_knn_stage_prepare_f32": [_vp, _vp, _i, _i, _i, _i, _i, _vp, _vp, _vp, _vp],
     "sonet_knn_stage_input_p16": [_vp, _vp, _vp, _vp, _vp, _i, _i, _i, _i, _i, _vp, _vp],
     "sonet_pointmlp_h3p_gmax": [_vp, _i, _vp, _i, _vp, _vp, _vp, _i, _i, _i, _i, _i, _i, _i, _vp, _vp, _vp],
+    "sonet_pointmlp_h3p_gmax_knn": [_vp, _vp, _i, _vp, _vp, _vp, _i, _vp, _vp, _vp, _i, _i, _i, _i, _i, _i, _vp, _vp],
     "sonet_node_stage_columns": [_i, _i],
     "sonet_p16_flat_to_bcm_f32": [_vp, _vp, _i, _i, _i, _vp],
     "sonet_som_sort_group_f32": [_vp, _vp, _vp, _vp, _vp, _i, _i, _i, _i, _vp, _vp, _vp, _vp, _vp, _vp, _vp, _vp],
diff --git a/so-net_amd/sonet_hip/ops.py b/so-net_amd/sonet_hip/ops.py
--- a/so-net_amd/sonet_hip/ops.py
+++ b/so-net_amd/sonet_hip/ops.py
@@ -727,6 +727,7 @@
 NODE_LINEAR_SPLIT = _os.environ.get("SONET_NODE_LINEAR_SPLIT", "1") != "0"
 P16_CHAINS = _os.environ.get("SONET_P16_CHAINS", "1") != "0"
 NODE_STAGE_P16 = _os.environ.get("SONET_NODE_STAGE_P16", "1") != "0"
+KNN_GMAX_FUSED = _os.environ.get("SONET_KNN_GMAX_FUSED", "1") != "0"
 POOLED_TRAIN_EPILOGUE = _os.environ.get("SONET_POOLED_TRAIN_EPILOGUE", "1") != "0"
 H3_SEGPOOL = _os.environ.get("SONET_H3_SEGPOOL", "1") != "0"
 H3_NORM_ON_LOAD = _os.environ.get("SONET_H3_NORM_ON_LOAD", "1") != "0"
@@ -1666,6 +1667,40 @@
         check(_lib.load().sonet_knn_stage_input_p16(ptr(prep["rec"]), ptr(z.data), ptr(wl), ptr(scale), ptr(shift), int(bool(relu)),
                                                     prep["B"], prep["M"], prep["K"], C, ptr(h1.data), stream_ptr()), "sonet_knn_stage_input_p16")
     return h1
+
+
+KNN_GMAX_FUSED_MAX_C = 512
+
+
+def knn_gmax_fused(prep, z, wl, scale1, shift1, relu1, wp, scale2, shift2, relu2, Cout, Lout):
+    B, M, K = prep["B"], prep["M"], prep["K"]
+    if not isinstance(z, P16) or z.B != 1 or z.L != node_stage_columns(B, M):
+        raise SonetHipError("knn_gmax_fused: z is a P16 1 x C x Lm activation")
+    C = z.C
+    if C > KNN_GMAX_FUSED_MAX_C:
+        raise SonetHipError("knn_gmax_fused: C=%d above %d" % (C, KNN_GMAX_FUSED_MAX_C))
+    for t, n in ((wl, "wl"), (scale1, "scale1"), (shift1, "shift1"), (scale2, "scale2"), (shift2, "shift2")):
+        _chk(t, n, torch.float32, 2 if n == "wl" else 1)
+    if tuple(wl.shape) != (C, 3) or scale1.numel() != C or shift1.numel() != C:
+        raise SonetHipError("knn_gmax_fused: wl C x 3, scale1 / shift1 C")
+    if wp.dtype != torch.int32:
+        raise SonetHipError("knn_gmax_fused: an h3p pack (ops.pointmlp_h3p_pack)")
+    if scale2.numel() != Cout or shift2.numel() != Cout:
+        raise SonetHipError("knn_gmax_fused: scale2 / shift2 Cout")
+    dev = _same_device(prep["rec"], z.data, wl, scale1, shift1, wp, scale2, shift2)
+    lib = _lib.load()
+    if wp.numel() * 4 != lib.sonet_pointmlp_h3p_pack_size(C, Cout):
+        raise SonetHipError("packed weight has %d bytes, expected %d for Cin=%d Cout=%d"
+                            % (wp.numel() * 4, lib.sonet_pointmlp_h3p_pack_size(C, Cout), C, Cout))
+    Lout = int(Lout)
+    yp = p16_flat(Cout, Lout, B * M, dev)
+    name = "pointmlph3p_gmax%d_knn_%dx%d_L%d" % (K, C, Cout, B * M * K)
+    _range_arm(name)
+    with _lib.on_device(dev), _timed(name):
+        check(lib.sonet_pointmlp_h3p_gmax_knn(ptr(prep["rec"]), ptr(z.data), C, ptr(wl), ptr(scale1), ptr(shift1), int(bool(relu1)), ptr(wp),
+                                              ptr(scale2), ptr(shift2), int(bool(relu2)), int(Cout), B, M, K, Lout, ptr(yp.data), stream_ptr()),
+              "sonet_pointmlp_h3p_gmax_knn")
+    return yp
 
 
 def p16_flat_to_bcm(p, B, M):
```
